# lixiny/ArtiBoost

Measured on AMD Instinct MI355X. Metric: synth samples/sec (render+fwd+bwd) 256x256 bs=64, higher is better.
Workload: dtype bf16x3; 1 GPU; train_artiboost HO3Dv2-clasbased (HybridBaseline/ResNet-34, 22x28x32x32 heat-map) + online CCV render 512->256, per-GPU batch 64, HO3D-like objects; global_batch=64, image=256, parallelism=dp1, graph=True, render_overlap=False

## Files before the change

artiboost_amd/csrc/conv_x3.hip:

```cpp
#include "conv_common.h"
#include "wgrad.h"

int conv3x3_x3_tiles(int N, int H, int W, int C, int Cn);
int conv3x3_x3_tiles_bnr(int N, int H, int W, int C, int Cn);
struct C3EvalBn { void* out_hi; void* out_lo; float* out_f32; const void* res_hi; const void* res_lo; int relu; };
int conv3x3_x3_run(const void* x_hi, const void* x_lo, const void* wt_hi, const void* wt_lo, float* out, int N, int H, int W,
                   int C, int Cn, int flip, const float* addend, float* stats, hipStream_t st, const float* bn_y = nullptr,
                   const void* bn_out_hi = nullptr, const float* bnp = nullptr, float* bn_part = nullptr, const C3EvalBn* ev = nullptr);
int conv_gemm2_x3_mtiles(int M, int Cn, int nsteps, int nclass);
int conv_gemm2_x3_run(ConvGemmArgs& g, hipStream_t st);
int conv_gemm2_x3_stem_mtiles(int M);
int conv_gemm2_x3_stem_run(ConvGemmArgs& g, hipStream_t st);
int stem_halo_x3_tiles(int N, int H, int W);
int stem_halo_x3_run(const void* xpad_hi, const void* xpad_lo, const void* w_hi, const void* w_lo, float* y, int N, int H, int W,
                     int Cout, float* stats, hipStream_t st);
int conv2x2_tfwd_rows(int N, int H, int W, int Cn, int K);
int conv2x2_tfwd_run(const void* x_hi, const void* x_lo, const void* wt_hi, const void* wt_lo, float* out, int N, int H, int W, int Cn, int K,
                     float* stats, hipStream_t st, const float* ep_scale = nullptr, const float* ep_shift = nullptr, int ep_relu = 0,
                     void* out_hi = nullptr, void* out_lo = nullptr);
int conv2x2_s2fwd_ok(int N, int H, int W, int C, int Cn);
int convp_s2fwd_rows(int N, int H, int W, int C, int Cn);
int convp_s2fwd_run(const void* x_hi, const void* x_lo, const void* w_hi, const void* w_lo, float* out, int N, int H, int W, int C, int Cn,
                    float* stats, hipStream_t st, const float* ep_scale = nullptr, const float* ep_shift = nullptr, int ep_relu = 0,
                    void* out_hi = nullptr, void* out_lo = nullptr);
// ... 316 lines not shown

extern "C" int ab_conv2d_wgrad_x3(const void* x_hi, const void* x_lo, const void* dy_hi, const void* dy_lo, float* dw, int N,
                                  int H, int W, int Cin, int Cout, int kh, int kw, int stride, int pad, void* workspace,
                                  int accumulate, void* stream) {
    if (!x_hi || !x_lo || !dy_hi || !dy_lo || !dw || !workspace) return AB_EINVAL;
    if (kh * kw > 16 || Cin % 64 || Cout % 64) return AB_ESHAPE;
    hipStream_t st = as_stream(stream);
    float* const slabs = (float*)workspace;
    const int jtot = kh * kw * Cin;
    if (x3_is_c3(kh, kw, stride, pad)) {
        if (int ns = wgrad3x3_x3_group_slices(1, N, H, W, Cin, Cout))
            return wgrad_then_reduce([&] { return wgrad3x3_x3_group_run(1, &x_hi, &x_lo, &dy_hi, &dy_lo, &slabs, N, H, W, Cin, Cout, st); },
                                     slabs, ns, Cout, jtot, jtot, dw, accumulate, 0, st);
    }
    {
        const long Ho = (H + 2 * pad - kh) / stride + 1, Wo = (W + 2 * pad - kw) / stride + 1;
        if ((long)N * Ho * Wo >= X3_WGRAD_MAX_M && N > 1) {
            const int n1 = N / 2;
            wgrad_reduce_now();
            const long xo = (long)n1 * H * W * Cin, yo = (long)n1 * Ho * Wo * Cout;
            int rc = ab_conv2d_wgrad_x3(x_hi, x_lo, dy_hi, dy_lo, dw, n1, H, W, Cin, Cout, kh, kw, stride, pad, workspace, accumulate, stream);
            if (rc) return rc;
            return ab_conv2d_wgrad_x3((const bf16_t*)x_hi + xo, (const bf16_t*)x_lo + xo, (const bf16_t*)dy_hi + yo, (const bf16_t*)dy_lo + yo,
                                      dw, N - n1, H, W, Cin, Cout, kh, kw, stride, pad, workspace, 1, stream);
        }
    }
    const int M = N * ((H + 2 * pad - kh) / stride + 1) * ((W + 2 * pad - kw) / stride + 1);
    int ns = wgrad_gemm2_x3_slices(M, Cout, Cin, kh * kw);
    if (ns <= 0) return AB_ESHAPE;
    return wgrad_then_reduce([&] { return wgrad_gemm2_x3_run(x_hi, x_lo, dy_hi, dy_lo, slabs, N, H, W, Cin, Cout, kh, kw, stride, pad, st); },
                             slabs, ns, Cout, jtot, jtot, dw, accumulate, 0, st);
}

extern "C" int ab_conv2d_stem_x3_stat_rows(int N, int H, int W) {
    if (int t = stem_halo_x3_tiles(N, H, W)) return t;
    return conv_gemm2_x3_stem_mtiles(N * (H / 2) * (W / 2));
}

extern "C" int ab_conv2d_stem_fwd_x3(const void* xpad_hi, const void* xpad_lo, const void* w_hi, const void* w_lo, float* y, int N,
                                     int H, int W, int Cout, float* stats, void* stream) {
    if (!xpad_hi || !w_hi || !w_lo || !y) return AB_EINVAL;
    if ((H & 1) || (W & 1) || Cout != 64) return AB_ESHAPE;
    if (stem_halo_x3_tiles(N, H, W)) return stem_halo_x3_run(xpad_hi, xpad_lo, w_hi, w_lo, y, N, H, W, Cout, stats, as_stream(stream));
    if (!xpad_lo) return AB_ESHAPE;
    ConvGemmArgs g = {};
    g.A = xpad_hi; g.A_lo = xpad_lo; g.Bw = w_hi; g.Bw_lo = w_lo; g.Out = y; g.stats = stats;
    g.N = N; g.Ha = H + 6; g.Wa = W + 8; g.Ca = 4;
    g.Ho = H / 2; g.Wo = W / 2; g.Cn = Cout; g.P = g.Ho; g.Q = g.Wo; g.out_sh = g.out_sw = 1; g.a_sh = g.a_sw = 2;
    g.ktot = 7 * 32; g.M = N * g.P * g.Q;
    return conv_gemm2_x3_stem_run(g, as_stream(stream));
}

static int stem_wgrad_x3_impl(const bf16_t* xpad_hi, const bf16_t* xpad_lo, const bf16_t* dy_hi, const bf16_t* dy_lo, float* dw, int N,
                              int H, int W, int Cout, void* workspace, int accumulate, hipStream_t st) {
    if ((long)N * (H / 2) * (W / 2) >= X3_WGRAD_MAX_M && N > 1) {
        const int n1 = N / 2;
        wgrad_reduce_now();
        const long xo = (long)n1 * (H + 6) * (W + 8) * 4, yo = (long)n1 * (H / 2) * (W / 2) * Cout;
        int rc = stem_wgrad_x3_impl(xpad_hi, xpad_lo, dy_hi, dy_lo, dw, n1, H, W, Cout, workspace, accumulate, st);
        if (rc) return rc;
        return stem_wgrad_x3_impl(xpad_hi + xo, xpad_lo ? xpad_lo + xo : nullptr, dy_hi + yo, dy_lo + yo, dw, N - n1, H, W, Cout, workspace, 1, st);
    }
    int ns = wgrad_gemm2_stem_slices(N, H, W, Cout);
    if (ns <= 0) return AB_ESHAPE;
    return wgrad_then_reduce([&] { return wgrad_gemm2_x3_stem_run(xpad_hi, xpad_lo, dy_hi, dy_lo, (float*)workspace, N, H, W, Cout, st); },
                             (float*)workspace, ns, Cout, 256, 7 * 32, dw, accumulate, 1, st);
// ... 10 lines not shown
```

artiboost_amd/csrc/torch_ops_gen.cpp:

```cpp
#include <ATen/ATen.h>
#include <c10/hip/HIPStream.h>
#include <torch/library.h>
#include "../../include/artiboost_hip.h"

static inline void* p(const c10::optional<at::Tensor>& t) { return (t.has_value() && t->defined()) ? t->data_ptr() : nullptr; }
static inline void* cur_stream() { return (void*)c10::hip::getCurrentHIPStream().stream(); }

#include <c10/hip/HIPFunctions.h>
typedef c10::optional<at::Tensor> OptT;
static inline bool has(const OptT& t) { return t.has_value() && t->defined(); }
static inline void ck_contig(const char* op, const char* a, const OptT& t) {
    if (has(t)) TORCH_CHECK(t->is_contiguous(), op, ": argument '", a, "' must be contiguous (the kernels take raw buffers)");
}
static inline void ck_dev(const char* op, const char* a, const OptT& t, int dt, bool contiguous) {
    if (!has(t)) return;
    TORCH_CHECK(t->is_cuda(), op, ": argument '", a, "' must be a HIP tensor, got a ", t->device().str(), " tensor");
    TORCH_CHECK(t->get_device() == c10::hip::current_device(), op, ": argument '", a, "' lives on device ", t->get_device(), ", the current device is ", (int)c10::hip::current_device());
    if (contiguous) TORCH_CHECK(t->is_contiguous(), op, ": argument '", a, "' must be contiguous (the kernel takes it as a raw buffer without a pitch)");
    if (dt >= 0) TORCH_CHECK((int)t->scalar_type() == dt, op, ": argument '", a, "' must be ", c10::toString((at::ScalarType)dt), ", got ", c10::toString(t->scalar_type()));
}
static inline void ck_host(const char* op, const char* a, const OptT& t) {
    if (!has(t)) return;
    TORCH_CHECK(t->is_cpu(), op, ": argument '", a, "' is a HOST structure / array of the C ABI and must be a CPU tensor, got a ", t->device().str(), " tensor");
    TORCH_CHECK(t->is_contiguous(), op, ": argument '", a, "' must be contiguous");
// ... 31 lines not shown
static void w_conv2d_stem_fwd(const c10::optional<at::Tensor>& xpad, const c10::optional<at::Tensor>& w, const c10::optional<at::Tensor>& y, int64_t dtype, int64_t N, int64_t H, int64_t W, int64_t Cout, const c10::optional<at::Tensor>& stats) { static const char* const OP = "artiboost_hip::conv2d_stem_fwd"; ck_dev(OP, "xpad", xpad, (int)-1, true); ck_dev(OP, "w", w, (int)-1, true); ck_dev(OP, "y", y, (int)-1, true); ck_dev(OP, "stats", stats, (int)at::kFloat, true); const long rc = (long)ab_conv2d_stem_fwd((const void*)p(xpad), (const void*)p(w), (void*)p(y), (int)dtype, (int)N, (int)H, (int)W, (int)Cout, (float*)p(stats), cur_stream()); TORCH_CHECK(rc == 0, "ab_conv2d_stem_fwd failed with code ", rc, rc > 0 ? " (hipError)" : " (argument error)"); }
static int64_t w_conv2d_dgrad_stat_rows(int64_t dtype, int64_t N, int64_t H, int64_t W, int64_t Cin, int64_t Cout, int64_t kh, int64_t kw, int64_t stride, int64_t pad) { return (int64_t)ab_conv2d_dgrad_stat_rows((int)dtype, (int)N, (int)H, (int)W, (int)Cin, (int)Cout, (int)kh, (int)kw, (int)stride, (int)pad); }
static void w_conv2d_dgrad(const c10::optional<at::Tensor>& dy, const c10::optional<at::Tensor>& wt, const c10::optional<at::Tensor>& dx, int64_t dtype, int64_t N, int64_t H, int64_t W, int64_t Cin, int64_t Cout, int64_t kh, int64_t kw, int64_t stride, int64_t pad, const c10::optional<at::Tensor>& addend, const c10::optional<at::Tensor>& stats) { static const char* const OP = "artiboost_hip::conv2d_dgrad"; ck_dev(OP, "dy", dy, (int)-1, true); ck_dev(OP, "wt", wt, (int)-1, true); ck_dev(OP, "dx", dx, (int)-1, true); ck_dev(OP, "addend", addend, (int)-1, true); ck_dev(OP, "stats", stats, (int)at::kFloat, true); ck_dtcode(OP, "dy", dy, dtype); ck_dtcode(OP, "wt", wt, dtype); ck_dtcode(OP, "dx", dx, dtype); ck_dtcode(OP, "addend", addend, dtype); ck_numel(OP, "dy", dy, (int64_t)(N*co(H,kh,stride,pad)*co(W,kw,stride,pad)*Cout)); ck_numel(OP, "wt", wt, (int64_t)(Cin*kh*kw*Cout)); ck_numel(OP, "dx", dx, (int64_t)(N*H*W*Cin)); ck_numel(OP, "addend", addend, (int64_t)(N*H*W*Cin)); const long rc = (long)ab_conv2d_dgrad((const void*)p(dy), (const void*)p(wt), (void*)p(dx), (int)dtype, (int)N, (int)H, (int)W, (int)Cin, (int)Cout, (int)kh, (int)kw, (int)stride, (int)pad, (const void*)p(addend), (float*)p(stats), cur_stream()); TORCH_CHECK(rc == 0, "ab_conv2d_dgrad failed with code ", rc, rc > 0 ? " (hipError)" : " (argument error)"); }
static int64_t w_conv2d_wgrad_workspace(int64_t M, int64_t Cout, int64_t jtot) { return (int64_t)ab_conv2d_wgrad_workspace((int)M, (int)Cout, (int)jtot); }
static void w_conv2d_wgrad(const c10::optional<at::Tensor>& x, const c10::optional<at::Tensor>& dy, const c10::optional<at::Tensor>& dw, int64_t dtype, int64_t N, int64_t H, int64_t W, int64_t Cin, int64_t Cout, int64_t kh, int64_t kw, int64_t stride, int64_t pad, const c10::optional<at::Tensor>& workspace, int64_t accumulate) { static const char* const OP = "artiboost_hip::conv2d_wgrad"; ck_dev(OP, "x", x, (int)-1, true); ck_dev(OP, "dy", dy, (int)-1, true); ck_dev(OP, "dw", dw, (int)at::kFloat, true); ck_dev(OP, "workspace", workspace, (int)-1, true); const long rc = (long)ab_conv2d_wgrad((const void*)p(x), (const void*)p(dy), (float*)p(dw), (int)dtype, (int)N, (int)H, (int)W, (int)Cin, (int)Cout, (int)kh, (int)kw, (int)stride, (int)pad, (void*)p(workspace), (int)accumulate, cur_stream()); TORCH_CHECK(rc == 0, "ab_conv2d_wgrad failed with code ", rc, rc > 0 ? " (hipError)" : " (argument error)"); }
static void w_conv2d_wgrad_deferred(const c10::optional<at::Tensor>& x, const c10::optional<at::Tensor>& dy, const c10::optional<at::Tensor>& dw, int64_t dtype, int64_t N, int64_t H, int64_t W, int64_t Cin, int64_t Cout, int64_t kh, int64_t kw, int64_t stride, int64_t pad, const c10::optional<at::Tensor>& workspace, int64_t accumulate, const c10::optional<at::Tensor>& pending) { static const char* const OP = "artiboost_hip::conv2d_wgrad_deferred"; ck_dev(OP, "x", x, (int)-1, true); ck_dev(OP, "dy", dy, (int)-1, true); ck_dev(OP, "dw", dw, (int)at::kFloat, true); ck_dev(OP, "workspace", workspace, (int)-1, true); ck_contig(OP, "pending", pending); const long rc = (long)ab_conv2d_wgrad_deferred((const void*)p(x), (const void*)p(dy), (float*)p(dw), (int)dtype, (int)N, (int)H, (int)W, (int)Cin, (int)Cout, (int)kh, (int)kw, (int)stride, (int)pad, (void*)p(workspace), (int)accumulate, (ab_wgrad_reduce_desc*)p(pending), cur_stream()); TORCH_CHECK(rc == 0, "ab_conv2d_wgrad_deferred failed with code ", rc, rc > 0 ? " (hipError)" : " (argument error)"); }
static void w_conv2d_stem_wgrad_deferred(const c10::optional<at::Tensor>& xpad, const c10::optional<at::Tensor>& dy, const c10::optional<at::Tensor>& dw, int64_t dtype, int64_t N, int64_t H, int64_t W, int64_t Cout, const c10::optional<at::Tensor>& workspace, const c10::optional<at::Tensor>& pending) { static const char* const OP = "artiboost_hip::conv2d_stem_wgrad_deferred"; ck_dev(OP, "xpad", xpad, (int)-1, true); ck_dev(OP, "dy", dy, (int)-1, true); ck_dev(OP, "dw", dw, (int)at::kFloat, true); ck_dev(OP, "workspace", workspace, (int)-1, true); ck_contig(OP, "pending", pending); const long rc = (long)ab_conv2d_stem_wgrad_deferred((const void*)p(xpad), (const void*)p(dy), (float*)p(dw), (int)dtype, (int)N, (int)H, (int)W, (int)Cout, (void*)p(workspace), (ab_wgrad_reduce_desc*)p(pending), cur_stream()); TORCH_CHECK(rc == 0, "ab_conv2d_stem_wgrad_deferred failed with code ", rc, rc > 0 ? " (hipError)" : " (argument error)"); }
static void w_conv2d_wgrad_x3_deferred(const c10::optional<at::Tensor>& x_hi, const c10::optional<at::Tensor>& x_lo, const c10::optional<at::Tensor>& dy_hi, const c10::optional<at::Tensor>& dy_lo, const c10::optional<at::Tensor>& dw, int64_t N, int64_t H, int64_t W, int64_t Cin, int64_t Cout, int64_t kh, int64_t kw, int64_t stride, int64_t pad, const c10::optional<at::Tensor>& workspace, int64_t accumulate, const c10::optional<at::Tensor>& pending) { static const char* const OP = "artiboost_hip::conv2d_wgrad_x3_deferred"; ck_dev(OP, "x_hi", x_hi, (int)-1, true); ck_dev(OP, "x_lo", x_lo, (int)-1, true); ck_dev(OP, "dy_hi", dy_hi, (int)-1, true); ck_dev(OP, "dy_lo", dy_lo, (int)-1, true); ck_dev(OP, "dw", dw, (int)at::kFloat, true); ck_dev(OP, "workspace", workspace, (int)-1, true); ck_contig(OP, "pending", pending); const long rc = (long)ab_conv2d_wgrad_x3_deferred((const void*)p(x_hi), (const void*)p(x_lo), (const void*)p(dy_hi), (const void*)p(dy_lo), (float*)p(dw), (int)N, (int)H, (int)W, (int)Cin, (int)Cout, (int)kh, (int)kw, (int)stride, (int)pad, (void*)p(workspace), (int)accumulate, (ab_wgrad_reduce_desc*)p(pending), cur_stream()); TORCH_CHECK(rc == 0, "ab_conv2d_wgrad_x3_deferred failed with code ", rc, rc > 0 ? " (hipError)" : " (argument error)"); }
static void w_conv2d_stem_wgrad_x3_deferred(const c10::optional<at::Tensor>& xpad_hi, const c10::optional<at::Tensor>& xpad_lo, const c10::optional<at::Tensor>& dy_hi, const c10::optional<at::Tensor>& dy_lo, const c10::optional<at::Tensor>& dw, int64_t N, int64_t H, int64_t W, int64_t Cout, const c10::optional<at::Tensor>& workspace, const c10::optional<at::Tensor>& pending) { static const char* const OP = "artiboost_hip::conv2d_stem_wgrad_x3_deferred"; ck_dev(OP, "xpad_hi", xpad_hi, (int)-1, true); ck_dev(OP, "xpad_lo", xpad_lo, (int)-1, true); ck_dev(OP, "dy_hi", dy_hi, (int)-1, true); ck_dev(OP, "dy_lo", dy_lo, (int)-1, true); ck_dev(OP, "dw", dw, (int)at::kFloat, true); ck_dev(OP, "workspace", workspace, (int)-1, true); ck_contig(OP, "pending", pending); const long rc = (long)ab_conv2d_stem_wgrad_x3_deferred((const void*)p(xpad_hi), (const void*)p(xpad_lo), (const void*)p(dy_hi), (const void*)p(dy_lo), (float*)p(dw), (int)N, (int)H, (int)W, (int)Cout, (void*)p(workspace), (ab_wgrad_reduce_desc*)p(pending), cur_stream()); TORCH_CHECK(rc == 0, "ab_conv2d_stem_wgrad_x3_deferred failed with code ", rc, rc > 0 ? " (hipError)" : " (argument error)"); }
static void w_wgrad_reduce_batch(const c10::optional<at::Tensor>& desc, int64_t n) { static const char* const OP = "artiboost_hip::wgrad_reduce_batch"; ck_contig(OP, "desc", desc); const long rc = (long)ab_wgrad_reduce_batch((const ab_wgrad_reduce_desc*)p(desc), (int)n, cur_stream()); TORCH_CHECK(rc == 0, "ab_wgrad_reduce_batch failed with code ", rc, rc > 0 ? " (hipError)" : " (argument error)"); }
static int64_t w_conv2d_wgrad_x3_group_workspace(int64_t G, int64_t N, int64_t H, int64_t W, int64_t Cin, int64_t Cout) { return (int64_t)ab_conv2d_wgrad_x3_group_workspace((int)G, (int)N, (int)H, (int)W, (int)Cin, (int)Cout); }
static void w_conv2d_wgrad_x3_group(const c10::optional<at::Tensor>& items_host, int64_t G, int64_t N, int64_t H, int64_t W, int64_t Cin, int64_t Cout, const c10::optional<at::Tensor>& workspace, int64_t accumulate) { static const char* const OP = "artiboost_hip::conv2d_wgrad_x3_group"; ck_host(OP, "items_host", items_host); ck_dev(OP, "workspace", workspace, (int)-1, true); ck_bytes(OP, "workspace", workspace, (int64_t)(ab_conv2d_wgrad_x3_group_workspace(G,N,H,W,Cin,Cout))); const long rc = (long)ab_conv2d_wgrad_x3_group((const ab_wgrad_group_item*)p(items_host), (int)G, (int)N, (int)H, (int)W, (int)Cin, (int)Cout, (void*)p(workspace), (int)accumulate, cur_stream()); TORCH_CHECK(rc == 0, "ab_conv2d_wgrad_x3_group failed with code ", rc, rc > 0 ? " (hipError)" : " (argument error)"); }
static int64_t w_conv2d_stem_wgrad_workspace(int64_t N, int64_t H, int64_t W, int64_t Cout) { return (int64_t)ab_conv2d_stem_wgrad_workspace((int)N, (int)H, (int)W, (int)Cout); }
static void w_conv2d_stem_wgrad(const c10::optional<at::Tensor>& xpad, const c10::optional<at::Tensor>& dy, const c10::optional<at::Tensor>& dw, int64_t dtype, int64_t N, int64_t H, int64_t W, int64_t Cout, const c10::optional<at::Tensor>& workspace) { static const char* const OP = "artiboost_hip::conv2d_stem_wgrad"; ck_dev(OP, "xpad", xpad, (int)-1, true); ck_dev(OP, "dy", dy, (int)-1, true); ck_dev(OP, "dw", dw, (int)at::kFloat, true); ck_dev(OP, "workspace", workspace, (int)-1, true); const long rc = (long)ab_conv2d_stem_wgrad((const void*)p(xpad), (const void*)p(dy), (float*)p(dw), (int)dtype, (int)N, (int)H, (int)W, (int)Cout, (void*)p(workspace), cur_stream()); TORCH_CHECK(rc == 0, "ab_conv2d_stem_wgrad failed with code ", rc, rc > 0 ? " (hipError)" : " (argument error)"); }
static void w_split_f32(const c10::optional<at::Tensor>& src, int64_t n, const c10::optional<at::Tensor>& hi, const c10::optional<at::Tensor>& lo) { static const char* const OP = "artiboost_hip::split_f32"; ck_dev(OP, "src", src, (int)at::kFloat, true); ck_dev(OP, "hi", hi, (int)-1, true); ck_dev(OP, "lo", lo, (int)-1, true); ck_dtype(OP, "hi", hi, at::kBFloat16); ck_dtype(OP, "lo", lo, at::kBFloat16); ck_numel(OP, "src", src, (int64_t)(n)); ck_numel(OP, "hi", hi, (int64_t)(n)); ck_numel(OP, "lo", lo, (int64_t)(n)); const long rc = (long)ab_split_f32((const float*)p(src), (long)n, (void*)p(hi), (void*)p(lo), cur_stream()); TORCH_CHECK(rc == 0, "ab_split_f32 failed with code ", rc, rc > 0 ? " (hipError)" : " (argument error)"); }
static int64_t w_conv2d_x3_stat_rows(int64_t N, int64_t H, int64_t W, int64_t Cin, int64_t Cout, int64_t kh, int64_t kw, int64_t stride, int64_t pad) { return (int64_t)ab_conv2d_x3_stat_rows((int)N, (int)H, (int)W, (int)Cin, (int)Cout, (int)kh, (int)kw, (int)stride, (int)pad); }
static void w_conv2d_fwd_x3(const c10::optional<at::Tensor>& x_hi, const c10::optional<at::Tensor>& x_lo, const c10::optional<at::Tensor>& w_hi, const c10::optional<at::Tensor>& w_lo, const c10::optional<at::Tensor>& y, int64_t N, int64_t H, int64_t W, int64_t Cin, int64_t Cout, int64_t kh, int64_t kw, int64_t stride, int64_t pad, const c10::optional<at::Tensor>& bias, const c10::optional<at::Tensor>& stats, int64_t relu) { static const char* const OP = "artiboost_hip::conv2d_fwd_x3"; ck_dev(OP, "x_hi", x_hi, (int)-1, true); ck_dev(OP, "x_lo", x_lo, (int)-1, true); ck_dev(OP, "w_hi", w_hi, (int)-1, true); ck_dev(OP, "w_lo", w_lo, (int)-1, true); ck_dev(OP, "y", y, (int)at::kFloat, true); ck_dev(OP, "bias", bias, (int)at::kFloat, true); ck_dev(OP, "stats", stats, (int)at::kFloat, true); ck_dtype(OP, "x_hi", x_hi, at::kBFloat16); ck_dtype(OP, "x_lo", x_lo, at::kBFloat16); ck_dtype(OP, "w_hi", w_hi, at::kBFloat16); ck_dtype(OP, "w_lo", w_lo, at::kBFloat16); ck_numel(OP, "x_hi", x_hi, (int64_t)(N*H*W*Cin)); ck_numel(OP, "x_lo", x_lo, (int64_t)(N*H*W*Cin)); ck_numel(OP, "w_hi", w_hi, (int64_t)(Cout*kh*kw*Cin)); ck_numel(OP, "w_lo", w_lo, (int64_t)(Cout*kh*kw*Cin)); ck_numel(OP, "y", y, (int64_t)(N*co(H,kh,stride,pad)*co(W,kw,stride,pad)*Cout)); ck_numel(OP, "bias", bias, (int64_t)(Cout)); ck_numel(OP, "stats", stats, (int64_t)(ab_conv2d_x3_stat_rows(N,H,W,Cin,Cout,kh,kw,stride,pad)*Cout*2)); const long rc = (long)ab_conv2d_fwd_x3((const void*)p(x_hi), (const void*)p(x_lo), (const void*)p(w_hi), (const void*)p(w_lo), (float*)p(y), (int)N, (int)H, (int)W, (int)Cin, (int)Cout, (int)kh, (int)kw, (int)stride, (int)pad, (const float*)p(bias), (float*)p(stats), (int)relu, cur_stream()); TORCH_CHECK(rc == 0, "ab_conv2d_fwd_x3 failed with code ", rc, rc > 0 ? " (hipError)" : " (argument error)"); }
static int64_t w_conv1x1_sam_fwd_x3_ok(int64_t B, int64_t H, int64_t W, int64_t Cin, int64_t C, int64_t D) { return (int64_t)ab_conv1x1_sam_fwd_x3_ok((int)B, (int)H, (int)W, (int)Cin, (int)C, (int)D); }
static void w_conv1x1_sam_fwd_x3(const c10::optional<at::Tensor>& x_hi, const c10::optional<at::Tensor>& x_lo, const c10::optional<at::Tensor>& w_hi, const c10::optional<at::Tensor>& w_lo, const c10::optional<at::Tensor>& bias, const c10::optional<at::Tensor>& logits, int64_t B, int64_t H, int64_t W, int64_t Cin, int64_t C, int64_t D, const c10::optional<at::Tensor>& part) { static const char* const OP = "artiboost_hip::conv1x1_sam_fwd_x3"; ck_dev(OP, "x_hi", x_hi, (int)-1, true); ck_dev(OP, "x_lo", x_lo, (int)-1, true); ck_dev(OP, "w_hi", w_hi, (int)-1, true); ck_dev(OP, "w_lo", w_lo, (int)-1, true); ck_dev(OP, "bias", bias, (int)at::kFloat, true); ck_dev(OP, "logits", logits, (int)at::kFloat, true); ck_dev(OP, "part", part, (int)at::kFloat, true); ck_dtype(OP, "x_hi", x_hi, at::kBFloat16); ck_dtype(OP, "x_lo", x_lo, at::kBFloat16); ck_dtype(OP, "w_hi", w_hi, at::kBFloat16); ck_dtype(OP, "w_lo", w_lo, at::kBFloat16); ck_numel(OP, "x_hi", x_hi, (int64_t)(B*H*W*Cin)); ck_numel(OP, "x_lo", x_lo, (int64_t)(B*H*W*Cin)); ck_numel(OP, "w_hi", w_hi, (int64_t)(C*32*Cin)); ck_numel(OP, "w_lo", w_lo, (int64_t)(C*32*Cin)); ck_numel(OP, "bias", bias, (int64_t)(C*32)); ck_numel(OP, "logits", logits, (int64_t)(B*H*W*C*32)); ck_numel(OP, "part", part, (int64_t)(B*(H*W/64)*C*8)); const long rc = (long)ab_conv1x1_sam_fwd_x3((const void*)p(x_hi), (const void*)p(x_lo), (const void*)p(w_hi), (const void*)p(w_lo), (const float*)p(bias), (float*)p(logits), (int)B, (int)H, (int)W, (int)Cin, (int)C, (int)D, (float*)p(part), cur_stream()); TORCH_CHECK(rc == 0, "ab_conv1x1_sam_fwd_x3 failed with code ", rc, rc > 0 ? " (hipError)" : " (argument error)"); }
static void w_softargmax3d_stage2(const c10::optional<at::Tensor>& part, int64_t B, int64_t C, int64_t ntile, const c10::optional<at::Tensor>& uvd, const c10::optional<at::Tensor>& conf, const c10::optional<at::Tensor>& stat) { static const char* const OP = "artiboost_hip::softargmax3d_stage2"; ck_dev(OP, "part", part, (int)at::kFloat, true); ck_dev(OP, "uvd", uvd, (int)at::kFloat, true); ck_dev(OP, "conf", conf, (int)at::kFloat, true); ck_dev(OP, "stat", stat, (int)at::kFloat, true); ck_numel(OP, "part", part, (int64_t)(B*ntile*C*8)); ck_numel(OP, "uvd", uvd, (int64_t)(B*C*3)); ck_numel(OP, "conf", conf, (int64_t)(B*C)); ck_numel(OP, "stat", stat, (int64_t)(B*C*2)); const long rc = (long)ab_softargmax3d_stage2((const float*)p(part), (int)B, (int)C, (int)ntile, (float*)p(uvd), (float*)p(conf), (float*)p(stat), cur_stream()); TORCH_CHECK(rc == 0, "ab_softargmax3d_stage2 failed with code ", rc, rc > 0 ? " (hipError)" : " (argument error)"); }
static int64_t w_conv2d_fwd_x3_evalbn_ok(int64_t N, int64_t H, int64_t W, int64_t Cin, int64_t Cout) { return (int64_t)ab_conv2d_fwd_x3_evalbn_ok((int)N, (int)H, (int)W, (int)Cin, (int)Cout); }
static void w_conv2d_fwd_x3_evalbn(const c10::optional<at::Tensor>& x_hi, const c10::optional<at::Tensor>& x_lo, const c10::optional<at::Tensor>& w_hi, const c10::optional<at::Tensor>& w_lo, int64_t N, int64_t H, int64_t W, int64_t Cin, int64_t Cout, const c10::optional<at::Tensor>& bnp, const c10::optional<at::Tensor>& res_hi, const c10::optional<at::Tensor>& res_lo, const c10::optional<at::Tensor>& res_f32, int64_t relu, const c10::optional<at::Tensor>& out_hi, const c10::optional<at::Tensor>& out_lo, const c10::optional<at::Tensor>& out_f32) { static const char* const OP = "artiboost_hip::conv2d_fwd_x3_evalbn"; ck_dev(OP, "x_hi", x_hi, (int)-1, true); ck_dev(OP, "x_lo", x_lo, (int)-1, true); ck_dev(OP, "w_hi", w_hi, (int)-1, true); ck_dev(OP, "w_lo", w_lo, (int)-1, true); ck_dev(OP, "bnp", bnp, (int)at::kFloat, true); ck_dev(OP, "res_hi", res_hi, (int)-1, true); ck_dev(OP, "res_lo", res_lo, (int)-1, true); ck_dev(OP, "res_f32", res_f32, (int)at::kFloat, true); ck_dev(OP, "out_hi", out_hi, (int)-1, true); ck_dev(OP, "out_lo", out_lo, (int)-1, true); ck_dev(OP, "out_f32", out_f32, (int)at::kFloat, true); ck_dtype(OP, "x_hi", x_hi, at::kBFloat16); ck_dtype(OP, "x_lo", x_lo, at::kBFloat16); ck_dtype(OP, "w_hi", w_hi, at::kBFloat16); ck_dtype(OP, "w_lo", w_lo, at::kBFloat16); ck_dtype(OP, "res_hi", res_hi, at::kBFloat16); ck_dtype(OP, "res_lo", res_lo, at::kBFloat16); ck_dtype(OP, "out_hi", out_hi, at::kBFloat16); ck_dtype(OP, "out_lo", out_lo, at::kBFloat16); ck_numel(OP, "x_hi", x_hi, (int64_t)(N*H*W*Cin)); ck_numel(OP, "x_lo", x_lo, (int64_t)(N*H*W*Cin)); ck_numel(OP, "w_hi", w_hi, (int64_t)(Cout*9*Cin)); ck_numel(OP, "w_lo", w_lo, (int64_t)(Cout*9*Cin)); ck_numel(OP, "bnp", bnp, (int64_t)(2*Cout)); ck_numel(OP, "res_hi", res_hi, (int64_t)(N*H*W*Cout)); ck_numel(OP, "res_lo", res_lo, (int64_t)(N*H*W*Cout)); ck_numel(OP, "res_f32", res_f32, (int64_t)(N*H*W*Cout)); ck_numel(OP, "out_hi", out_hi, (int64_t)(N*H*W*Cout)); ck_numel(OP, "out_lo", out_lo, (int64_t)(N*H*W*Cout)); ck_numel(OP, "out_f32", out_f32, (int64_t)(N*H*W*Cout)); const long rc = (long)ab_conv2d_fwd_x3_evalbn((const void*)p(x_hi), (const void*)p(x_lo), (const void*)p(w_hi), (const void*)p(w_lo), (int)N, (int)H, (int)W, (int)Cin, (int)Cout, (const float*)p(bnp), (const void*)p(res_hi), (const void*)p(res_lo), (const float*)p(res_f32), (int)relu, (void*)p(out_hi), (void*)p(out_lo), (float*)p(out_f32), cur_stream()); TORCH_CHECK(rc == 0, "ab_conv2d_fwd_x3_evalbn failed with code ", rc, rc > 0 ? " (hipError)" : " (argument error)"); }
static void w_conv2d_fwd_x3_affine(const c10::optional<at::Tensor>& x_hi, const c10::optional<at::Tensor>& x_lo, const c10::optional<at::Tensor>& w_hi, const c10::optional<at::Tensor>& w_lo, int64_t N, int64_t H, int64_t W, int64_t Cin, int64_t Cout, int64_t kh, int64_t kw, int64_t stride, int64_t pad, const c10::optional<at::Tensor>& scale, const c10::optional<at::Tensor>& shift, int64_t relu, const c10::optional<at::Tensor>& out_f32, const c10::optional<at::Tensor>& out_hi, const c10::optional<at::Tensor>& out_lo) { static const char* const OP = "artiboost_hip::conv2d_fwd_x3_affine"; ck_dev(OP, "x_hi", x_hi, (int)-1, true); ck_dev(OP, "x_lo", x_lo, (int)-1, true); ck_dev(OP, "w_hi", w_hi, (int)-1, true); ck_dev(OP, "w_lo", w_lo, (int)-1, true); ck_dev(OP, "scale", scale, (int)at::kFloat, true); ck_dev(OP, "shift", shift, (int)at::kFloat, true); ck_dev(OP, "out_f32", out_f32, (int)at::kFloat, true); ck_dev(OP, "out_hi", out_hi, (int)-1, true); ck_dev(OP, "out_lo", out_lo, (int)-1, true); ck_dtype(OP, "x_hi", x_hi, at::kBFloat16); ck_dtype(OP, "x_lo", x_lo, at::kBFloat16); ck_dtype(OP, "w_hi", w_hi, at::kBFloat16); ck_dtype(OP, "w_lo", w_lo, at::kBFloat16); ck_dtype(OP, "out_hi", out_hi, at::kBFloat16); ck_dtype(OP, "out_lo", out_lo, at::kBFloat16); ck_numel(OP, "x_hi", x_hi, (int64_t)(N*H*W*Cin)); ck_numel(OP, "x_lo", x_lo, (int64_t)(N*H*W*Cin)); ck_numel(OP, "w_hi", w_hi, (int64_t)(Cout*kh*kw*Cin)); ck_numel(OP, "w_lo", w_lo, (int64_t)(Cout*kh*kw*Cin)); ck_numel(OP, "scale", scale, (int64_t)(Cout)); ck_numel(OP, "shift", shift, (int64_t)(Cout)); ck_numel(OP, "out_f32", out_f32, (int64_t)(N*co(H,kh,stride,pad)*co(W,kw,stride,pad)*Cout)); ck_numel(OP, "out_hi", out_hi, (int64_t)(N*co(H,kh,stride,pad)*co(W,kw,stride,pad)*Cout)); ck_numel(OP, "out_lo", out_lo, (int64_t)(N*co(H,kh,stride,pad)*co(W,kw,stride,pad)*Cout)); const long rc = (long)ab_conv2d_fwd_x3_affine((const void*)p(x_hi), (const void*)p(x_lo), (const void*)p(w_hi), (const void*)p(w_lo), (int)N, (int)H, (int)W, (int)Cin, (int)Cout, (int)kh, (int)kw, (int)stride, (int)pad, (const float*)p(scale), (const float*)p(shift), (int)relu, (float*)p(out_f32), (void*)p(out_hi), (void*)p(out_lo), cur_stream()); TORCH_CHECK(rc == 0, "ab_conv2d_fwd_x3_affine failed with code ", rc, rc > 0 ? " (hipError)" : " (argument error)"); }
static void w_conv2d_dgrad_x3_affine(const c10::optional<at::Tensor>& dy_hi, const c10::optional<at::Tensor>& dy_lo, const c10::optional<at::Tensor>& wt_hi, const c10::optional<at::Tensor>& wt_lo, int64_t N, int64_t H, int64_t W, int64_t Cin, int64_t Cout, int64_t kh, int64_t kw, int64_t stride, int64_t pad, const c10::optional<at::Tensor>& scale, const c10::optional<at::Tensor>& shift, int64_t relu, const c10::optional<at::Tensor>& out_f32, const c10::optional<at::Tensor>& out_hi, const c10::optional<at::Tensor>& out_lo) { static const char* const OP = "artiboost_hip::conv2d_dgrad_x3_affine"; ck_dev(OP, "dy_hi", dy_hi, (int)-1, true); ck_dev(OP, "dy_lo", dy_lo, (int)-1, true); ck_dev(OP, "wt_hi", wt_hi, (int)-1, true); ck_dev(OP, "wt_lo", wt_lo, (int)-1, true); ck_dev(OP, "scale", scale, (int)at::kFloat, true); ck_dev(OP, "shift", shift, (int)at::kFloat, true); ck_dev(OP, "out_f32", out_f32, (int)at::kFloat, true); ck_dev(OP, "out_hi", out_hi, (int)-1, true); ck_dev(OP, "out_lo", out_lo, (int)-1, true); const long rc = (long)ab_conv2d_dgrad_x3_affine((const void*)p(dy_hi), (const void*)p(dy_lo), (const void*)p(wt_hi), (const void*)p(wt_lo), (int)N, (int)H, (int)W, (int)Cin, (int)Cout, (int)kh, (int)kw, (int)stride, (int)pad, (const float*)p(scale), (const float*)p(shift), (int)relu, (float*)p(out_f32), (void*)p(out_hi), (void*)p(out_lo), cur_stream()); TORCH_CHECK(rc == 0, "ab_conv2d_dgrad_x3_affine failed with code ", rc, rc > 0 ? " (hipError)" : " (argument error)"); }
static int64_t w_conv2d_dgrad_x3_stat_rows(int64_t N, int64_t H, int64_t W, int64_t Cin, int64_t Cout, int64_t kh, int64_t kw, int64_t stride, int64_t pad) { return (int64_t)ab_conv2d_dgrad_x3_stat_rows((int)N, (int)H, (int)W, (int)Cin, (int)Cout, (int)kh, (int)kw, (int)stride, (int)pad); }
static void w_conv2d_dgrad_x3(const c10::optional<at::Tensor>& dy_hi, const c10::optional<at::Tensor>& dy_lo, const c10::optional<at::Tensor>& wt_hi, const c10::optional<at::Tensor>& wt_lo, const c10::optional<at::Tensor>& dx, int64_t N, int64_t H, int64_t W, int64_t Cin, int64_t Cout, int64_t kh, int64_t kw, int64_t stride, int64_t pad, const c10::optional<at::Tensor>& addend, const c10::optional<at::Tensor>& stats) { static const char* const OP = "artiboost_hip::conv2d_dgrad_x3"; ck_dev(OP, "dy_hi", dy_hi, (int)-1, true); ck_dev(OP, "dy_lo", dy_lo, (int)-1, true); ck_dev(OP, "wt_hi", wt_hi, (int)-1, true); ck_dev(OP, "wt_lo", wt_lo, (int)-1, true); ck_dev(OP, "dx", dx, (int)at::kFloat, true); ck_dev(OP, "addend", addend, (int)at::kFloat, true); ck_dev(OP, "stats", stats, (int)at::kFloat, true); ck_dtype(OP, "dy_hi", dy_hi, at::kBFloat16); ck_dtype(OP, "dy_lo", dy_lo, at::kBFloat16); ck_dtype(OP, "wt_hi", wt_hi, at::kBFloat16); ck_dtype(OP, "wt_lo", wt_lo, at::kBFloat16); ck_numel(OP, "dy_hi", dy_hi, (int64_t)(N*co(H,kh,stride,pad)*co(W,kw,stride,pad)*Cout)); ck_numel(OP, "dy_lo", dy_lo, (int64_t)(N*co(H,kh,stride,pad)*co(W,kw,stride,pad)*Cout)); ck_numel(OP, "wt_hi", wt_hi, (int64_t)(Cin*kh*kw*Cout)); ck_numel(OP, "wt_lo", wt_lo, (int64_t)(Cin*kh*kw*Cout)); ck_numel(OP, "dx", dx, (int64_t)(N*H*W*Cin)); ck_numel(OP, "addend", addend, (int64_t)(N*H*W*Cin)); const long rc = (long)ab_conv2d_dgrad_x3((const void*)p(dy_hi), (const void*)p(dy_lo), (const void*)p(wt_hi), (const void*)p(wt_lo), (float*)p(dx), (int)N, (int)H, (int)W, (int)Cin, (int)Cout, (int)kh, (int)kw, (int)stride, (int)pad, (const float*)p(addend), (float*)p(stats), cur_stream()); TORCH_CHECK(rc == 0, "ab_conv2d_dgrad_x3 failed with code ", rc, rc > 0 ? " (hipError)" : " (argument error)"); }
static void w_conv2d_dgrad_x3_pair(const c10::optional<at::Tensor>& dy_hi, const c10::optional<at::Tensor>& dy_lo, const c10::optional<at::Tensor>& wt_hi, const c10::optional<at::Tensor>& wt_lo, const c10::optional<at::Tensor>& dy2_hi, const c10::optional<at::Tensor>& dy2_lo, const c10::optional<at::Tensor>& wt2_hi, const c10::optional<at::Tensor>& wt2_lo, const c10::optional<at::Tensor>& dx, int64_t N, int64_t H, int64_t W, int64_t Cin, int64_t Cout, int64_t kh, int64_t kw, int64_t pad, const c10::optional<at::Tensor>& addend) { static const char* const OP = "artiboost_hip::conv2d_dgrad_x3_pair"; ck_dev(OP, "dy_hi", dy_hi, (int)-1, true); ck_dev(OP, "dy_lo", dy_lo, (int)-1, true); ck_dev(OP, "wt_hi", wt_hi, (int)-1, true); ck_dev(OP, "wt_lo", wt_lo, (int)-1, true); ck_dev(OP, "dy2_hi", dy2_hi, (int)-1, true); ck_dev(OP, "dy2_lo", dy2_lo, (int)-1, true); ck_dev(OP, "wt2_hi", wt2_hi, (int)-1, true); ck_dev(OP, "wt2_lo", wt2_lo, (int)-1, true); ck_dev(OP, "dx", dx, (int)at::kFloat, true); ck_dev(OP, "addend", addend, (int)at::kFloat, true); ck_dtype(OP, "dy_hi", dy_hi, at::kBFloat16); ck_dtype(OP, "dy_lo", dy_lo, at::kBFloat16); ck_dtype(OP, "wt_hi", wt_hi, at::kBFloat16); ck_dtype(OP, "wt_lo", wt_lo, at::kBFloat16); ck_dtype(OP, "dy2_hi", dy2_hi, at::kBFloat16); ck_dtype(OP, "dy2_lo", dy2_lo, at::kBFloat16); ck_dtype(OP, "wt2_hi", wt2_hi, at::kBFloat16); ck_dtype(OP, "wt2_lo", wt2_lo, at::kBFloat16); ck_numel(OP, "dy_hi", dy_hi, (int64_t)(N*(H/2)*(W/2)*Cout)); ck_numel(OP, "dy_lo", dy_lo, (int64_t)(N*(H/2)*(W/2)*Cout)); ck_numel(OP, "dy2_hi", dy2_hi, (int64_t)(N*(H/2)*(W/2)*Cout)); ck_numel(OP, "dy2_lo", dy2_lo, (int64_t)(N*(H/2)*(W/2)*Cout)); ck_numel(OP, "wt_hi", wt_hi, (int64_t)(Cin*kh*kw*Cout)); ck_numel(OP, "wt_lo", wt_lo, (int64_t)(Cin*kh*kw*Cout)); ck_numel(OP, "wt2_hi", wt2_hi, (int64_t)(Cin*Cout)); ck_numel(OP, "wt2_lo", wt2_lo, (int64_t)(Cin*Cout)); ck_numel(OP, "dx", dx, (int64_t)(N*H*W*Cin)); ck_numel(OP, "addend", addend, (int64_t)(N*H*W*Cin)); const long rc = (long)ab_conv2d_dgrad_x3_pair((const void*)p(dy_hi), (const void*)p(dy_lo), (const void*)p(wt_hi), (const void*)p(wt_lo), (const void*)p(dy2_hi), (const void*)p(dy2_lo), (const void*)p(wt2_hi), (const void*)p(wt2_lo), (float*)p(dx), (int)N, (int)H, (int)W, (int)Cin, (int)Cout, (int)kh, (int)kw, (int)pad, (const float*)p(addend), cur_stream()); TORCH_CHECK(rc == 0, "ab_conv2d_dgrad_x3_pair failed with code ", rc, rc > 0 ? " (hipError)" : " (argument error)"); }
static int64_t w_conv2d_dgrad_x3_pair_bn_rows(int64_t N, int64_t H, int64_t W, int64_t Cin, int64_t Cout, int64_t kh, int64_t kw, int64_t pad) { return (int64_t)ab_conv2d_dgrad_x3_pair_bn_rows((int)N, (int)H, (int)W, (int)Cin, (int)Cout, (int)kh, (int)kw, (int)pad); }
static void w_conv2d_dgrad_x3_pair_bn(const c10::optional<at::Tensor>& dy_hi, const c10::optional<at::Tensor>& dy_lo, const c10::optional<at::Tensor>& wt_hi, const c10::optional<at::Tensor>& wt_lo, const c10::optional<at::Tensor>& dy2_hi, const c10::optional<at::Tensor>& dy2_lo, const c10::optional<at::Tensor>& wt2_hi, const c10::optional<at::Tensor>& wt2_lo, const c10::optional<at::Tensor>& dz, int64_t N, int64_t H, int64_t W, int64_t Cin, int64_t Cout, int64_t kh, int64_t kw, int64_t pad, const c10::optional<at::Tensor>& bn_y, const c10::optional<at::Tensor>& bn_out_hi, const c10::optional<at::Tensor>& bnp, const c10::optional<at::Tensor>& bn_part) { static const char* const OP = "artiboost_hip::conv2d_dgrad_x3_pair_bn"; ck_dev(OP, "dy_hi", dy_hi, (int)-1, true); ck_dev(OP, "dy_lo", dy_lo, (int)-1, true); ck_dev(OP, "wt_hi", wt_hi, (int)-1, true); ck_dev(OP, "wt_lo", wt_lo, (int)-1, true); ck_dev(OP, "dy2_hi", dy2_hi, (int)-1, true); ck_dev(OP, "dy2_lo", dy2_lo, (int)-1, true); ck_dev(OP, "wt2_hi", wt2_hi, (int)-1, true); ck_dev(OP, "wt2_lo", wt2_lo, (int)-1, true); ck_dev(OP, "dz", dz, (int)at::kFloat, true); ck_dev(OP, "bn_y", bn_y, (int)at::kFloat, true); ck_dev(OP, "bn_out_hi", bn_out_hi, (int)-1, true); ck_dev(OP, "bnp", bnp, (int)at::kFloat, true); ck_dev(OP, "bn_part", bn_part, (int)at::kFloat, true); ck_dtype(OP, "dy_hi", dy_hi, at::kBFloat16); ck_dtype(OP, "dy_lo", dy_lo, at::kBFloat16); ck_dtype(OP, "wt_hi", wt_hi, at::kBFloat16); ck_dtype(OP, "wt_lo", wt_lo, at::kBFloat16); ck_dtype(OP, "dy2_hi", dy2_hi, at::kBFloat16); ck_dtype(OP, "dy2_lo", dy2_lo, at::kBFloat16); ck_dtype(OP, "wt2_hi", wt2_hi, at::kBFloat16); ck_dtype(OP, "wt2_lo", wt2_lo, at::kBFloat16); ck_dtype(OP, "bn_out_hi", bn_out_hi, at::kBFloat16); ck_numel(OP, "dy_hi", dy_hi, (int64_t)(N*(H/2)*(W/2)*Cout)); ck_numel(OP, "dy_lo", dy_lo, (int64_t)(N*(H/2)*(W/2)*Cout)); ck_numel(OP, "dy2_hi", dy2_hi, (int64_t)(N*(H/2)*(W/2)*Cout)); ck_numel(OP, "dy2_lo", dy2_lo, (int64_t)(N*(H/2)*(W/2)*Cout)); ck_numel(OP, "wt_hi", wt_hi, (int64_t)(Cin*kh*kw*Cout)); ck_numel(OP, "wt_lo", wt_lo, (int64_t)(Cin*kh*kw*Cout)); ck_numel(OP, "wt2_hi", wt2_hi, (int64_t)(Cin*Cout)); ck_numel(OP, "wt2_lo", wt2_lo, (int64_t)(Cin*Cout)); ck_numel(OP, "dz", dz, (int64_t)(N*H*W*Cin)); ck_numel(OP, "bn_y", bn_y, (int64_t)(N*H*W*Cin)); ck_numel(OP, "bn_out_hi", bn_out_hi, (int64_t)(N*H*W*Cin)); ck_numel(OP, "bnp", bnp, (int64_t)(4*Cin)); ck_numel(OP, "bn_part", bn_part, (int64_t)(ab_conv2d_dgrad_x3_pair_bn_rows(N,H,W,Cin,Cout,kh,kw,pad)*Cin*2)); const long rc = (long)ab_conv2d_dgrad_x3_pair_bn((const void*)p(dy_hi), (const void*)p(dy_lo), (const void*)p(wt_hi), (const void*)p(wt_lo), (const void*)p(dy2_hi), (const void*)p(dy2_lo), (const void*)p(wt2_hi), (const void*)p(wt2_lo), (float*)p(dz), (int)N, (int)H, (int)W, (int)Cin, (int)Cout, (int)kh, (int)kw, (int)pad, (const float*)p(bn_y), (const void*)p(bn_out_hi), (const float*)p(bnp), (float*)p(bn_part), cur_stream()); TORCH_CHECK(rc == 0, "ab_conv2d_dgrad_x3_pair_bn failed with code ", rc, rc > 0 ? " (hipError)" : " (argument error)"); }
static int64_t w_conv2d_dgrad_x3_bn_rows(int64_t N, int64_t H, int64_t W, int64_t Cin, int64_t Cout, int64_t kh, int64_t kw, int64_t stride, int64_t pad) { return (int64_t)ab_conv2d_dgrad_x3_bn_rows((int)N, (int)H, (int)W, (int)Cin, (int)Cout, (int)kh, (int)kw, (int)stride, (int)pad); }
static void w_conv2d_dgrad_x3_bn(const c10::optional<at::Tensor>& dy_hi, const c10::optional<at::Tensor>& dy_lo, const c10::optional<at::Tensor>& wt_hi, const c10::optional<at::Tensor>& wt_lo, const c10::optional<at::Tensor>& dz, int64_t N, int64_t H, int64_t W, int64_t Cin, int64_t Cout, int64_t kh, int64_t kw, int64_t stride, int64_t pad, const c10::optional<at::Tensor>& addend, const c10::optional<at::Tensor>& bn_y, const c10::optional<at::Tensor>& bn_out_hi, const c10::optional<at::Tensor>& bnp, const c10::optional<at::Tensor>& bn_part) { static const char* const OP = "artiboost_hip::conv2d_dgrad_x3_bn"; ck_dev(OP, "dy_hi", dy_hi, (int)-1, true); ck_dev(OP, "dy_lo", dy_lo, (int)-1, true); ck_dev(OP, "wt_hi", wt_hi, (int)-1, true); ck_dev(OP, "wt_lo", wt_lo, (int)-1, true); ck_dev(OP, "dz", dz, (int)at::kFloat, true); ck_dev(OP, "addend", addend, (int)at::kFloat, true); ck_dev(OP, "bn_y", bn_y, (int)at::kFloat, true); ck_dev(OP, "bn_out_hi", bn_out_hi, (int)-1, true); ck_dev(OP, "bnp", bnp, (int)at::kFloat, true); ck_dev(OP, "bn_part", bn_part, (int)at::kFloat, true); ck_dtype(OP, "dy_hi", dy_hi, at::kBFloat16); ck_dtype(OP, "dy_lo", dy_lo, at::kBFloat16); ck_dtype(OP, "wt_hi", wt_hi, at::kBFloat16); ck_dtype(OP, "wt_lo", wt_lo, at::kBFloat16); ck_dtype(OP, "bn_out_hi", bn_out_hi, at::kBFloat16); ck_numel(OP, "dy_hi", dy_hi, (int64_t)(N*co(H,kh,stride,pad)*co(W,kw,stride,pad)*Cout)); ck_numel(OP, "dy_lo", dy_lo, (int64_t)(N*co(H,kh,stride,pad)*co(W,kw,stride,pad)*Cout)); ck_numel(OP, "wt_hi", wt_hi, (int64_t)(Cin*kh*kw*Cout)); ck_numel(OP, "wt_lo", wt_lo, (int64_t)(Cin*kh*kw*Cout)); ck_numel(OP, "dz", dz, (int64_t)(N*H*W*Cin)); ck_numel(OP, "addend", addend, (int64_t)(N*H*W*Cin)); ck_numel(OP, "bn_y", bn_y, (int64_t)(N*H*W*Cin)); ck_numel(OP, "bn_out_hi", bn_out_hi, (int64_t)(N*H*W*Cin)); ck_numel(OP, "bnp", bnp, (int64_t)(4*Cin)); ck_numel(OP, "bn_part", bn_part, (int64_t)(ab_conv2d_dgrad_x3_bn_rows(N,H,W,Cin,Cout,kh,kw,stride,pad)*Cin*2)); const long rc = (long)ab_conv2d_dgrad_x3_bn((const void*)p(dy_hi), (const void*)p(dy_lo), (const void*)p(wt_hi), (const void*)p(wt_lo), (float*)p(dz), (int)N, (int)H, (int)W, (int)Cin, (int)Cout, (int)kh, (int)kw, (int)stride, (int)pad, (const float*)p(addend), (const float*)p(bn_y), (const void*)p(bn_out_hi), (const float*)p(bnp), (float*)p(bn_part), cur_stream()); TORCH_CHECK(rc == 0, "ab_conv2d_dgrad_x3_bn failed with code ", rc, rc > 0 ? " (hipError)" : " (argument error)"); }
static int64_t w_conv2d_wgrad_x3_workspace(int64_t N, int64_t H, int64_t W, int64_t Cin, int64_t Cout, int64_t kh, int64_t kw, int64_t stride, int64_t pad) { return (int64_t)ab_conv2d_wgrad_x3_workspace((int)N, (int)H, (int)W, (int)Cin, (int)Cout, (int)kh, (int)kw, (int)stride, (int)pad); }
static void w_conv2d_wgrad_x3(const c10::optional<at::Tensor>& x_hi, const c10::optional<at::Tensor>& x_lo, const c10::optional<at::Tensor>& dy_hi, const c10::optional<at::Tensor>& dy_lo, const c10::optional<at::Tensor>& dw, int64_t N, int64_t H, int64_t W, int64_t Cin, int64_t Cout, int64_t kh, int64_t kw, int64_t stride, int64_t pad, const c10::optional<at::Tensor>& workspace, int64_t accumulate) { static const char* const OP = "artiboost_hip::conv2d_wgrad_x3"; ck_dev(OP, "x_hi", x_hi, (int)-1, true); ck_dev(OP, "x_lo", x_lo, (int)-1, true); ck_dev(OP, "dy_hi", dy_hi, (int)-1, true); ck_dev(OP, "dy_lo", dy_lo, (int)-1, true); ck_dev(OP, "dw", dw, (int)at::kFloat, true); ck_dev(OP, "workspace", workspace, (int)-1, true); ck_dtype(OP, "x_hi", x_hi, at::kBFloat16); ck_dtype(OP, "x_lo", x_lo, at::kBFloat16); ck_dtype(OP, "dy_hi", dy_hi, at::kBFloat16); ck_dtype(OP, "dy_lo", dy_lo, at::kBFloat16); ck_numel(OP, "x_hi", x_hi, (int64_t)(N*H*W*Cin)); ck_numel(OP, "x_lo", x_lo, (int64_t)(N*H*W*Cin)); ck_numel(OP, "dy_hi", dy_hi, (int64_t)(N*co(H,kh,stride,pad)*co(W,kw,stride,pad)*Cout)); ck_numel(OP, "dy_lo", dy_lo, (int64_t)(N*co(H,kh,stride,pad)*co(W,kw,stride,pad)*Cout)); ck_numel(OP, "dw", dw, (int64_t)(Cout*kh*kw*Cin)); ck_bytes(OP, "workspace", workspace, (int64_t)(ab_conv2d_wgrad_x3_workspace(N,H,W,Cin,Cout,kh,kw,stride,pad))); const long rc = (long)ab_conv2d_wgrad_x3((const void*)p(x_hi), (const void*)p(x_lo), (const void*)p(dy_hi), (const void*)p(dy_lo), (float*)p(dw), (int)N, (int)H, (int)W, (int)Cin, (int)Cout, (int)kh, (int)kw, (int)stride, (int)pad, (void*)p(workspace), (int)accumulate, cur_stream()); TORCH_CHECK(rc == 0, "ab_conv2d_wgrad_x3 failed with code ", rc, rc > 0 ? " (hipError)" : " (argument error)"); }
static int64_t w_conv2d_stem_x3_stat_rows(int64_t N, int64_t H, int64_t W) { return (int64_t)ab_conv2d_stem_x3_stat_rows((int)N, (int)H, (int)W); }
static void w_conv2d_stem_fwd_x3(const c10::optional<at::Tensor>& xpad_hi, const c10::optional<at::Tensor>& xpad_lo, const c10::optional<at::Tensor>& w_hi, const c10::optional<at::Tensor>& w_lo, const c10::optional<at::Tensor>& y, int64_t N, int64_t H, int64_t W, int64_t Cout, const c10::optional<at::Tensor>& stats) { static const char* const OP = "artiboost_hip::conv2d_stem_fwd_x3"; ck_dev(OP, "xpad_hi", xpad_hi, (int)-1, true); ck_dev(OP, "xpad_lo", xpad_lo, (int)-1, true); ck_dev(OP, "w_hi", w_hi, (int)-1, true); ck_dev(OP, "w_lo", w_lo, (int)-1, true); ck_dev(OP, "y", y, (int)at::kFloat, true); ck_dev(OP, "stats", stats, (int)at::kFloat, true); ck_dtype(OP, "xpad_hi", xpad_hi, at::kBFloat16); ck_dtype(OP, "xpad_lo", xpad_lo, at::kBFloat16); ck_dtype(OP, "w_hi", w_hi, at::kBFloat16); ck_dtype(OP, "w_lo", w_lo, at::kBFloat16); ck_numel(OP, "xpad_hi", xpad_hi, (int64_t)(N*(H+6)*(W+8)*4)); ck_numel(OP, "xpad_lo", xpad_lo, (int64_t)(N*(H+6)*(W+8)*4)); ck_numel(OP, "w_hi", w_hi, (int64_t)(Cout*7*8*4)); ck_numel(OP, "w_lo", w_lo, (int64_t)(Cout*7*8*4)); ck_numel(OP, "y", y, (int64_t)(N*(H/2)*(W/2)*Cout)); ck_numel(OP, "stats", stats, (int64_t)(ab_conv2d_stem_x3_stat_rows(N,H,W)*Cout*2)); const long rc = (long)ab_conv2d_stem_fwd_x3((const void*)p(xpad_hi), (const void*)p(xpad_lo), (const void*)p(w_hi), (const void*)p(w_lo), (float*)p(y), (int)N, (int)H, (int)W, (int)Cout, (float*)p(stats), cur_stream()); TORCH_CHECK(rc == 0, "ab_conv2d_stem_fwd_x3 failed with code ", rc, rc > 0 ? " (hipError)" : " (argument error)"); }
static void w_conv2d_stem_wgrad_x3(const c10::optional<at::Tensor>& xpad_hi, const c10::optional<at::Tensor>& xpad_lo, const c10::optional<at::Tensor>& dy_hi, const c10::optional<at::Tensor>& dy_lo, const c10::optional<at::Tensor>& dw, int64_t N, int64_t H, int64_t W, int64_t Cout, const c10::optional<at::Tensor>& workspace) { static const char* const OP = "artiboost_hip::conv2d_stem_wgrad_x3"; ck_dev(OP, "xpad_hi", xpad_hi, (int)-1, true); ck_dev(OP, "xpad_lo", xpad_lo, (int)-1, true); ck_dev(OP, "dy_hi", dy_hi, (int)-1, true); ck_dev(OP, "dy_lo", dy_lo, (int)-1, true); ck_dev(OP, "dw", dw, (int)at::kFloat, true); ck_dev(OP, "workspace", workspace, (int)-1, true); ck_dtype(OP, "xpad_hi", xpad_hi, at::kBFloat16); ck_dtype(OP, "xpad_lo", xpad_lo, at::kBFloat16); ck_dtype(OP, "dy_hi", dy_hi, at::kBFloat16); ck_dtype(OP, "dy_lo", dy_lo, at::kBFloat16); ck_numel(OP, "xpad_hi", xpad_hi, (int64_t)(N*(H+6)*(W+8)*4)); ck_numel(OP, "xpad_lo", xpad_lo, (int64_t)(N*(H+6)*(W+8)*4)); ck_numel(OP, "dy_hi", dy_hi, (int64_t)(N*(H/2)*(W/2)*Cout)); ck_numel(OP, "dy_lo", dy_lo, (int64_t)(N*(H/2)*(W/2)*Cout)); ck_numel(OP, "dw", dw, (int64_t)(Cout*7*8*4)); const long rc = (long)ab_conv2d_stem_wgrad_x3((const void*)p(xpad_hi), (const void*)p(xpad_lo), (const void*)p(dy_hi), (const void*)p(dy_lo), (float*)p(dw), (int)N, (int)H, (int)W, (int)Cout, (void*)p(workspace), cur_stream()); TORCH_CHECK(rc == 0, "ab_conv2d_stem_wgrad_x3 failed with code ", rc, rc > 0 ? " (hipError)" : " (argument error)"); }
static void w_bn_apply_x3(const c10::optional<at::Tensor>& y, const c10::optional<at::Tensor>& res, const c10::optional<at::Tensor>& bnp, int64_t M, int64_t C, int64_t relu, const c10::optional<at::Tensor>& out, const c10::optional<at::Tensor>& out_hi, const c10::optional<at::Tensor>& out_lo) { static const char* const OP = "artiboost_hip::bn_apply_x3"; ck_dev(OP, "y", y, (int)at::kFloat, true); ck_dev(OP, "res", res, (int)at::kFloat, true); ck_dev(OP, "bnp", bnp, (int)at::kFloat, true); ck_dev(OP, "out", out, (int)at::kFloat, true); ck_dev(OP, "out_hi", out_hi, (int)-1, true); ck_dev(OP, "out_lo", out_lo, (int)-1, true); ck_dtype(OP, "out_hi", out_hi, at::kBFloat16); ck_dtype(OP, "out_lo", out_lo, at::kBFloat16); ck_numel(OP, "y", y, (int64_t)(M*C)); ck_numel(OP, "res", res, (int64_t)(M*C)); ck_numel(OP, "out", out, (int64_t)(M*C)); ck_numel(OP, "out_hi", out_hi, (int64_t)(M*C)); ck_numel(OP, "out_lo", out_lo, (int64_t)(M*C)); ck_numel(OP, "bnp", bnp, (int64_t)(2*C)); const long rc = (long)ab_bn_apply_x3((const float*)p(y), (const float*)p(res), (const float*)p(bnp), (long)M, (int)C, (int)relu, (float*)p(out), (void*)p(out_hi), (void*)p(out_lo), cur_stream()); TORCH_CHECK(rc == 0, "ab_bn_apply_x3 failed with code ", rc, rc > 0 ? " (hipError)" : " (argument error)"); }
static void w_bn_apply_x3_resbn(const c10::optional<at::Tensor>& y, const c10::optional<at::Tensor>& res_y, const c10::optional<at::Tensor>& bnp, const c10::optional<at::Tensor>& res_bnp, int64_t M, int64_t C, int64_t relu, const c10::optional<at::Tensor>& out, const c10::optional<at::Tensor>& out_hi, const c10::optional<at::Tensor>& out_lo) { static const char* const OP = "artiboost_hip::bn_apply_x3_resbn"; ck_dev(OP, "y", y, (int)at::kFloat, true); ck_dev(OP, "res_y", res_y, (int)at::kFloat, true); ck_dev(OP, "bnp", bnp, (int)at::kFloat, true); ck_dev(OP, "res_bnp", res_bnp, (int)at::kFloat, true); ck_dev(OP, "out", out, (int)at::kFloat, true); ck_dev(OP, "out_hi", out_hi, (int)-1, true); ck_dev(OP, "out_lo", out_lo, (int)-1, true); const long rc = (long)ab_bn_apply_x3_resbn((const float*)p(y), (const float*)p(res_y), (const float*)p(bnp), (const float*)p(res_bnp), (long)M, (int)C, (int)relu, (float*)p(out), (void*)p(out_hi), (void*)p(out_lo), cur_stream()); TORCH_CHECK(rc == 0, "ab_bn_apply_x3_resbn failed with code ", rc, rc > 0 ? " (hipError)" : " (argument error)"); }
static void w_bn_apply_x3_respl(const c10::optional<at::Tensor>& y, const c10::optional<at::Tensor>& res_hi, const c10::optional<at::Tensor>& res_lo, const c10::optional<at::Tensor>& bnp, int64_t M, int64_t C, int64_t relu, const c10::optional<at::Tensor>& out, const c10::optional<at::Tensor>& out_hi, const c10::optional<at::Tensor>& out_lo) { static const char* const OP = "artiboost_hip::bn_apply_x3_respl"; ck_dev(OP, "y", y, (int)at::kFloat, true); ck_dev(OP, "res_hi", res_hi, (int)-1, true); ck_dev(OP, "res_lo", res_lo, (int)-1, true); ck_dev(OP, "bnp", bnp, (int)at::kFloat, true); ck_dev(OP, "out", out, (int)at::kFloat, true); ck_dev(OP, "out_hi", out_hi, (int)-1, true); ck_dev(OP, "out_lo", out_lo, (int)-1, true); ck_dtype(OP, "res_hi", res_hi, at::kBFloat16); ck_dtype(OP, "res_lo", res_lo, at::kBFloat16); ck_dtype(OP, "out_hi", out_hi, at::kBFloat16); ck_dtype(OP, "out_lo", out_lo, at::kBFloat16); ck_numel(OP, "y", y, (int64_t)(M*C)); ck_numel(OP, "res_hi", res_hi, (int64_t)(M*C)); ck_numel(OP, "res_lo", res_lo, (int64_t)(M*C)); ck_numel(OP, "out", out, (int64_t)(M*C)); ck_numel(OP, "out_hi", out_hi, (int64_t)(M*C)); ck_numel(OP, "out_lo", out_lo, (int64_t)(M*C)); ck_numel(OP, "bnp", bnp, (int64_t)(2*C)); const long rc = (long)ab_bn_apply_x3_respl((const float*)p(y), (const void*)p(res_hi), (const void*)p(res_lo), (const float*)p(bnp), (long)M, (int)C, (int)relu, (float*)p(out), (void*)p(out_hi), (void*)p(out_lo), cur_stream()); TORCH_CHECK(rc == 0, "ab_bn_apply_x3_respl failed with code ", rc, rc > 0 ? " (hipError)" : " (argument error)"); }
static int64_t w_bn_fin_apply_x3_ok(int64_t nparts, int64_t C) { return (int64_t)ab_bn_fin_apply_x3_ok((int)nparts, (int)C); }
static void w_bn_fin_apply_x3(const c10::optional<at::Tensor>& part, int64_t nparts, int64_t count, const c10::optional<at::Tensor>& gamma, const c10::optional<at::Tensor>& beta, double eps, double momentum, const c10::optional<at::Tensor>& running_mean, const c10::optional<at::Tensor>& running_var, const c10::optional<at::Tensor>& bnp, const c10::optional<at::Tensor>& y, const c10::optional<at::Tensor>& res, const c10::optional<at::Tensor>& res_hi, const c10::optional<at::Tensor>& res_lo, const c10::optional<at::Tensor>& res_bnp, int64_t M, int64_t C, int64_t relu, const c10::optional<at::Tensor>& out, const c10::optional<at::Tensor>& out_hi, const c10::optional<at::Tensor>& out_lo) { static const char* const OP = "artiboost_hip::bn_fin_apply_x3"; ck_dev(OP, "part", part, (int)at::kFloat, true); ck_dev(OP, "gamma", gamma, (int)at::kFloat, true); ck_dev(OP, "beta", beta, (int)at::kFloat, true); ck_dev(OP, "running_mean", running_mean, (int)at::kFloat, true); ck_dev(OP, "running_var", running_var, (int)at::kFloat, true); ck_dev(OP, "bnp", bnp, (int)at::kFloat, true); ck_dev(OP, "y", y, (int)at::kFloat, true); ck_dev(OP, "res", res, (int)at::kFloat, true); ck_dev(OP, "res_hi", res_hi, (int)-1, true); ck_dev(OP, "res_lo", res_lo, (int)-1, true); ck_dev(OP, "res_bnp", res_bnp, (int)at::kFloat, true); ck_dev(OP, "out", out, (int)at::kFloat, true); ck_dev(OP, "out_hi", out_hi, (int)-1, true); ck_dev(OP, "out_lo", out_lo, (int)-1, true); ck_dtype(OP, "res_hi", res_hi, at::kBFloat16); ck_dtype(OP, "res_lo", res_lo, at::kBFloat16); ck_dtype(OP, "out_hi", out_hi, at::kBFloat16); ck_dtype(OP, "out_lo", out_lo, at::kBFloat16); ck_numel(OP, "part", part, (int64_t)(nparts*C*2)); ck_numel(OP, "gamma", gamma, (int64_t)(C)); ck_numel(OP, "beta", beta, (int64_t)(C)); ck_numel(OP, "running_mean", running_mean, (int64_t)(C)); ck_numel(OP, "running_var", running_var, (int64_t)(C)); ck_numel(OP, "bnp", bnp, (int64_t)(4*C)); ck_numel(OP, "res_bnp", res_bnp, (int64_t)(2*C)); ck_numel(OP, "y", y, (int64_t)(M*C)); ck_numel(OP, "res", res, (int64_t)(M*C)); ck_numel(OP, "res_hi", res_hi, (int64_t)(M*C)); ck_numel(OP, "res_lo", res_lo, (int64_t)(M*C)); ck_numel(OP, "out", out, (int64_t)(M*C)); ck_numel(OP, "out_hi", out_hi, (int64_t)(M*C)); ck_numel(OP, "out_lo", out_lo, (int64_t)(M*C)); const long rc = (long)ab_bn_fin_apply_x3((const float*)p(part), (int)nparts, (long)count, (const float*)p(gamma), (const float*)p(beta), (float)eps, (float)momentum, (float*)p(running_mean), (float*)p(running_var), (float*)p(bnp), (const float*)p(y), (const float*)p(res), (const void*)p(res_hi), (const void*)p(res_lo), (const float*)p(res_bnp), (long)M, (int)C, (int)relu, (float*)p(out), (void*)p(out_hi), (void*)p(out_lo), cur_stream()); TORCH_CHECK(rc == 0, "ab_bn_fin_apply_x3 failed with code ", rc, rc > 0 ? " (hipError)" : " (argument error)"); }
static void w_bn_bwd_x3(const c10::optional<at::Tensor>& dout, const c10::optional<at::Tensor>& out, int64_t out_is_hi_plane, const c10::optional<at::Tensor>& y, const c10::optional<at::Tensor>& bnp, int64_t M, int64_t C, int64_t relu, const c10::optional<at::Tensor>& part, int64_t nparts_given, const c10::optional<at::Tensor>& bwdp, const c10::optional<at::Tensor>& dgamma, const c10::optional<at::Tensor>& dbeta, const c10::optional<at::Tensor>& dy_hi, const c10::optional<at::Tensor>& dy_lo, const c10::optional<at::Tensor>& dz_out) { static const char* const OP = "artiboost_hip::bn_bwd_x3"; ck_dev(OP, "dout", dout, (int)at::kFloat, true); ck_dev(OP, "out", out, (int)-1, true); ck_dev(OP, "y", y, (int)at::kFloat, true); ck_dev(OP, "bnp", bnp, (int)at::kFloat, true); ck_dev(OP, "part", part, (int)at::kFloat, true); ck_dev(OP, "bwdp", bwdp, (int)at::kFloat, true); ck_dev(OP, "dgamma", dgamma, (int)at::kFloat, true); ck_dev(OP, "dbeta", dbeta, (int)at::kFloat, true); ck_dev(OP, "dy_hi", dy_hi, (int)-1, true); ck_dev(OP, "dy_lo", dy_lo, (int)-1, true); ck_dev(OP, "dz_out", dz_out, (int)at::kFloat, true); ck_dtype(OP, "dy_hi", dy_hi, at::kBFloat16); ck_dtype(OP, "dy_lo", dy_lo, at::kBFloat16); ck_numel(OP, "dout", dout, (int64_t)(M*C)); ck_numel(OP, "y", y, (int64_t)(M*C)); ck_numel(OP, "dy_hi", dy_hi, (int64_t)(M*C)); ck_numel(OP, "dy_lo", dy_lo, (int64_t)(M*C)); ck_numel(OP, "dz_out", dz_out, (int64_t)(M*C)); ck_numel(OP, "bnp", bnp, (int64_t)(4*C)); ck_numel(OP, "dgamma", dgamma, (int64_t)(C)); ck_numel(OP, "dbeta", dbeta, (int64_t)(C)); const long rc = (long)ab_bn_bwd_x3((const float*)p(dout), (const void*)p(out), (int)out_is_hi_plane, (const float*)p(y), (const float*)p(bnp), (long)M, (int)C, (int)relu, (float*)p(part), (int)nparts_given, (float*)p(bwdp), (float*)p(dgamma), (float*)p(dbeta), (void*)p(dy_hi), (void*)p(dy_lo), (float*)p(dz_out), cur_stream()); TORCH_CHECK(rc == 0, "ab_bn_bwd_x3 failed with code ", rc, rc > 0 ? " (hipError)" : " (argument error)"); }
static int64_t w_col_stats_nparts(int64_t M) { return (int64_t)ab_col_stats_nparts((long)M); }
static void w_col_stats(const c10::optional<at::Tensor>& x, int64_t dtype, int64_t M, int64_t C, const c10::optional<at::Tensor>& part) { static const char* const OP = "artiboost_hip::col_stats"; ck_dev(OP, "x", x, (int)-1, true); ck_dev(OP, "part", part, (int)at::kFloat, true); ck_dtcode(OP, "x", x, dtype); ck_numel(OP, "x", x, (int64_t)(M*C)); ck_numel(OP, "part", part, (int64_t)(ab_col_stats_nparts(M)*C*2)); const long rc = (long)ab_col_stats((const void*)p(x), (int)dtype, (long)M, (int)C, (float*)p(part), cur_stream()); TORCH_CHECK(rc == 0, "ab_col_stats failed with code ", rc, rc > 0 ? " (hipError)" : " (argument error)"); }
static void w_bn_finalize(const c10::optional<at::Tensor>& part, int64_t nparts, int64_t C, int64_t count, const c10::optional<at::Tensor>& gamma, const c10::optional<at::Tensor>& beta, double eps, double momentum, const c10::optional<at::Tensor>& running_mean, const c10::optional<at::Tensor>& running_var, const c10::optional<at::Tensor>& bnp) { static const char* const OP = "artiboost_hip::bn_finalize"; ck_dev(OP, "part", part, (int)at::kFloat, true); ck_dev(OP, "gamma", gamma, (int)at::kFloat, true); ck_dev(OP, "beta", beta, (int)at::kFloat, true); ck_dev(OP, "running_mean", running_mean, (int)at::kFloat, true); ck_dev(OP, "running_var", running_var, (int)at::kFloat, true); ck_dev(OP, "bnp", bnp, (int)at::kFloat, true); ck_numel(OP, "part", part, (int64_t)(nparts*C*2)); ck_numel(OP, "gamma", gamma, (int64_t)(C)); ck_numel(OP, "beta", beta, (int64_t)(C)); ck_numel(OP, "running_mean", running_mean, (int64_t)(C)); ck_numel(OP, "running_var", running_var, (int64_t)(C)); ck_numel(OP, "bnp", bnp, (int64_t)(4*C)); const long rc = (long)ab_bn_finalize((const float*)p(part), (int)nparts, (int)C, (long)count, (const float*)p(gamma), (const float*)p(beta), (float)eps, (float)momentum, (float*)p(running_mean), (float*)p(running_var), (float*)p(bnp), cur_stream()); TORCH_CHECK(rc == 0, "ab_bn_finalize failed with code ", rc, rc > 0 ? " (hipError)" : " (argument error)"); }
static void w_bn_eval_params(int64_t C, const c10::optional<at::Tensor>& gamma, const c10::optional<at::Tensor>& beta, const c10::optional<at::Tensor>& rm, const c10::optional<at::Tensor>& rv, double eps, const c10::optional<at::Tensor>& bnp) { static const char* const OP = "artiboost_hip::bn_eval_params"; ck_dev(OP, "gamma", gamma, (int)at::kFloat, true); ck_dev(OP, "beta", beta, (int)at::kFloat, true); ck_dev(OP, "rm", rm, (int)at::kFloat, true); ck_dev(OP, "rv", rv, (int)at::kFloat, true); ck_dev(OP, "bnp", bnp, (int)at::kFloat, true); ck_numel(OP, "gamma", gamma, (int64_t)(C)); ck_numel(OP, "beta", beta, (int64_t)(C)); ck_numel(OP, "rm", rm, (int64_t)(C)); ck_numel(OP, "rv", rv, (int64_t)(C)); ck_numel(OP, "bnp", bnp, (int64_t)(4*C)); const long rc = (long)ab_bn_eval_params((int)C, (const float*)p(gamma), (const float*)p(beta), (const float*)p(rm), (const float*)p(rv), (float)eps, (float*)p(bnp), cur_stream()); TORCH_CHECK(rc == 0, "ab_bn_eval_params failed with code ", rc, rc > 0 ? " (hipError)" : " (argument error)"); }
static void w_bn_eval_params_batch(const c10::optional<at::Tensor>& flat, const c10::optional<at::Tensor>& stats, const c10::optional<at::Tensor>& desc_dev, int64_t n, int64_t max_c, double eps, const c10::optional<at::Tensor>& out) { static const char* const OP = "artiboost_hip::bn_eval_params_batch"; ck_dev(OP, "flat", flat, (int)at::kFloat, true); ck_dev(OP, "stats", stats, (int)at::kFloat, true); ck_dev(OP, "desc_dev", desc_dev, (int)at::kInt, true); ck_dev(OP, "out", out, (int)at::kFloat, true); const long rc = (long)ab_bn_eval_params_batch((const float*)p(flat), (const float*)p(stats), (const int32_t*)p(desc_dev), (int)n, (int)max_c, (float)eps, (float*)p(out), cur_stream()); TORCH_CHECK(rc == 0, "ab_bn_eval_params_batch failed with code ", rc, rc > 0 ? " (hipError)" : " (argument error)"); }
static void w_bn_apply(const c10::optional<at::Tensor>& y, const c10::optional<at::Tensor>& res, const c10::optional<at::Tensor>& bnp, int64_t dtype, int64_t M, int64_t C, int64_t relu, const c10::optional<at::Tensor>& out) { static const char* const OP = "artiboost_hip::bn_apply"; ck_dev(OP, "y", y, (int)-1, true); ck_dev(OP, "res", res, (int)-1, true); ck_dev(OP, "bnp", bnp, (int)at::kFloat, true); ck_dev(OP, "out", out, (int)-1, true); const long rc = (long)ab_bn_apply((const void*)p(y), (const void*)p(res), (const float*)p(bnp), (int)dtype, (long)M, (int)C, (int)relu, (void*)p(out), cur_stream()); TORCH_CHECK(rc == 0, "ab_bn_apply failed with code ", rc, rc > 0 ? " (hipError)" : " (argument error)"); }
static void w_bn_bwd(const c10::optional<at::Tensor>& dout, const c10::optional<at::Tensor>& out, const c10::optional<at::Tensor>& y, const c10::optional<at::Tensor>& bnp, int64_t dtype, int64_t M, int64_t C, int64_t relu, const c10::optional<at::Tensor>& part, const c10::optional<at::Tensor>& bwdp, const c10::optional<at::Tensor>& dgamma, const c10::optional<at::Tensor>& dbeta, const c10::optional<at::Tensor>& dy, const c10::optional<at::Tensor>& dz_out) { static const char* const OP = "artiboost_hip::bn_bwd"; ck_dev(OP, "dout", dout, (int)-1, true); ck_dev(OP, "out", out, (int)-1, true); ck_dev(OP, "y", y, (int)-1, true); ck_dev(OP, "bnp", bnp, (int)at::kFloat, true); ck_dev(OP, "part", part, (int)at::kFloat, true); ck_dev(OP, "bwdp", bwdp, (int)at::kFloat, true); ck_dev(OP, "dgamma", dgamma, (int)at::kFloat, true); ck_dev(OP, "dbeta", dbeta, (int)at::kFloat, true); ck_dev(OP, "dy", dy, (int)-1, true); ck_dev(OP, "dz_out", dz_out, (int)-1, true); const long rc = (long)ab_bn_bwd((const void*)p(dout), (const void*)p(out), (const void*)p(y), (const float*)p(bnp), (int)dtype, (long)M, (int)C, (int)relu, (float*)p(part), (float*)p(bwdp), (float*)p(dgamma), (float*)p(dbeta), (void*)p(dy), (void*)p(dz_out), cur_stream()); TORCH_CHECK(rc == 0, "ab_bn_bwd failed with code ", rc, rc > 0 ? " (hipError)" : " (argument error)"); }
static void w_relu_bwd(const c10::optional<at::Tensor>& dout, const c10::optional<at::Tensor>& out, int64_t dtype, int64_t n, const c10::optional<at::Tensor>& dz) { static const char* const OP = "artiboost_hip::relu_bwd"; ck_dev(OP, "dout", dout, (int)-1, true); ck_dev(OP, "out", out, (int)-1, true); ck_dev(OP, "dz", dz, (int)-1, true); const long rc = (long)ab_relu_bwd((const void*)p(dout), (const void*)p(out), (int)dtype, (long)n, (void*)p(dz), cur_stream()); TORCH_CHECK(rc == 0, "ab_relu_bwd failed with code ", rc, rc > 0 ? " (hipError)" : " (argument error)"); }
static void w_col_sum(const c10::optional<at::Tensor>& x, int64_t dtype, int64_t M, int64_t C, const c10::optional<at::Tensor>& part, const c10::optional<at::Tensor>& out) { static const char* const OP = "artiboost_hip::col_sum"; ck_dev(OP, "x", x, (int)-1, true); ck_dev(OP, "part", part, (int)at::kFloat, true); ck_dev(OP, "out", out, (int)at::kFloat, true); const long rc = (long)ab_col_sum((const void*)p(x), (int)dtype, (long)M, (int)C, (float*)p(part), (float*)p(out), cur_stream()); TORCH_CHECK(rc == 0, "ab_col_sum failed with code ", rc, rc > 0 ? " (hipError)" : " (argument error)"); }
static void w_col_sum_x3(const c10::optional<at::Tensor>& hi, const c10::optional<at::Tensor>& lo, int64_t M, int64_t C, const c10::optional<at::Tensor>& part, const c10::optional<at::Tensor>& out) { static const char* const OP = "artiboost_hip::col_sum_x3"; ck_dev(OP, "hi", hi, (int)-1, true); ck_dev(OP, "lo", lo, (int)-1, true); ck_dev(OP, "part", part, (int)at::kFloat, true); ck_dev(OP, "out", out, (int)at::kFloat, true); const long rc = (long)ab_col_sum_x3((const void*)p(hi), (const void*)p(lo), (long)M, (int)C, (float*)p(part), (float*)p(out), cur_stream()); TORCH_CHECK(rc == 0, "ab_col_sum_x3 failed with code ", rc, rc > 0 ? " (hipError)" : " (argument error)"); }
static void w_add(const c10::optional<at::Tensor>& a, const c10::optional<at::Tensor>& b, int64_t dtype, int64_t n, const c10::optional<at::Tensor>& out) { static const char* const OP = "artiboost_hip::add"; ck_dev(OP, "a", a, (int)-1, true); ck_dev(OP, "b", b, (int)-1, true); ck_dev(OP, "out", out, (int)-1, true); const long rc = (long)ab_add((const void*)p(a), (const void*)p(b), (int)dtype, (long)n, (void*)p(out), cur_stream()); TORCH_CHECK(rc == 0, "ab_add failed with code ", rc, rc > 0 ? " (hipError)" : " (argument error)"); }
static void w_maxpool3x3s2_fwd(const c10::optional<at::Tensor>& x, int64_t dtype, int64_t N, int64_t H, int64_t W, int64_t C, const c10::optional<at::Tensor>& out, const c10::optional<at::Tensor>& idx) { static const char* const OP = "artiboost_hip::maxpool3x3s2_fwd"; ck_dev(OP, "x", x, (int)-1, true); ck_dev(OP, "out", out, (int)-1, true); ck_dev(OP, "idx", idx, (int)-1, true); const long rc = (long)ab_maxpool3x3s2_fwd((const void*)p(x), (int)dtype, (int)N, (int)H, (int)W, (int)C, (void*)p(out), (void*)p(idx), cur_stream()); TORCH_CHECK(rc == 0, "ab_maxpool3x3s2_fwd failed with code ", rc, rc > 0 ? " (hipError)" : " (argument error)"); }
static int64_t w_conv2d_dgrad_bnstats_rows(int64_t dtype, int64_t N, int64_t H, int64_t W, int64_t Cin, int64_t Cout, int64_t kh, int64_t kw, int64_t stride, int64_t pad) { return (int64_t)ab_conv2d_dgrad_bnstats_rows((int)dtype, (int)N, (int)H, (int)W, (int)Cin, (int)Cout, (int)kh, (int)kw, (int)stride, (int)pad); }
static void w_conv2d_dgrad_bnstats(const c10::optional<at::Tensor>& dy, const c10::optional<at::Tensor>& wt, const c10::optional<at::Tensor>& dx, int64_t dtype, int64_t N, int64_t H, int64_t W, int64_t Cin, int64_t Cout, int64_t kh, int64_t kw, int64_t stride, int64_t pad, const c10::optional<at::Tensor>& addend, const c10::optional<at::Tensor>& bn_y, const c10::optional<at::Tensor>& bn_out, const c10::optional<at::Tensor>& bnp, const c10::optional<at::Tensor>& bn_part) { static const char* const OP = "artiboost_hip::conv2d_dgrad_bnstats"; ck_dev(OP, "dy", dy, (int)-1, true); ck_dev(OP, "wt", wt, (int)-1, true); ck_dev(OP, "dx", dx, (int)-1, true); ck_dev(OP, "addend", addend, (int)-1, true); ck_dev(OP, "bn_y", bn_y, (int)-1, true); ck_dev(OP, "bn_out", bn_out, (int)-1, true); ck_dev(OP, "bnp", bnp, (int)at::kFloat, true); ck_dev(OP, "bn_part", bn_part, (int)at::kFloat, true); const long rc = (long)ab_conv2d_dgrad_bnstats((const void*)p(dy), (const void*)p(wt), (void*)p(dx), (int)dtype, (int)N, (int)H, (int)W, (int)Cin, (int)Cout, (int)kh, (int)kw, (int)stride, (int)pad, (const void*)p(addend), (const void*)p(bn_y), (const void*)p(bn_out), (const float*)p(bnp), (float*)p(bn_part), cur_stream()); TORCH_CHECK(rc == 0, "ab_conv2d_dgrad_bnstats failed with code ", rc, rc > 0 ? " (hipError)" : " (argument error)"); }
static void w_bn_bwd_apply(const c10::optional<at::Tensor>& dout, const c10::optional<at::Tensor>& out, const c10::optional<at::Tensor>& y, const c10::optional<at::Tensor>& bnp, int64_t dtype, int64_t M, int64_t C, int64_t relu, const c10::optional<at::Tensor>& part, int64_t nparts, const c10::optional<at::Tensor>& bwdp, const c10::optional<at::Tensor>& dgamma, const c10::optional<at::Tensor>& dbeta, const c10::optional<at::Tensor>& dy, const c10::optional<at::Tensor>& dz_out) { static const char* const OP = "artiboost_hip::bn_bwd_apply"; ck_dev(OP, "dout", dout, (int)-1, true); ck_dev(OP, "out", out, (int)-1, true); ck_dev(OP, "y", y, (int)-1, true); ck_dev(OP, "bnp", bnp, (int)at::kFloat, true); ck_dev(OP, "part", part, (int)at::kFloat, true); ck_dev(OP, "bwdp", bwdp, (int)at::kFloat, true); ck_dev(OP, "dgamma", dgamma, (int)at::kFloat, true); ck_dev(OP, "dbeta", dbeta, (int)at::kFloat, true); ck_dev(OP, "dy", dy, (int)-1, true); ck_dev(OP, "dz_out", dz_out, (int)-1, true); const long rc = (long)ab_bn_bwd_apply((const void*)p(dout), (const void*)p(out), (const void*)p(y), (const float*)p(bnp), (int)dtype, (long)M, (int)C, (int)relu, (const float*)p(part), (int)nparts, (float*)p(bwdp), (float*)p(dgamma), (float*)p(dbeta), (void*)p(dy), (void*)p(dz_out), cur_stream()); TORCH_CHECK(rc == 0, "ab_bn_bwd_apply failed with code ", rc, rc > 0 ? " (hipError)" : " (argument error)"); }
static void w_bn_relu_maxpool3x3s2_fwd(const c10::optional<at::Tensor>& y, const c10::optional<at::Tensor>& bnp, int64_t dtype, int64_t N, int64_t H, int64_t W, int64_t C, const c10::optional<at::Tensor>& out, const c10::optional<at::Tensor>& idx) { static const char* const OP = "artiboost_hip::bn_relu_maxpool3x3s2_fwd"; ck_dev(OP, "y", y, (int)-1, true); ck_dev(OP, "bnp", bnp, (int)at::kFloat, true); ck_dev(OP, "out", out, (int)-1, true); ck_dev(OP, "idx", idx, (int)-1, true); const long rc = (long)ab_bn_relu_maxpool3x3s2_fwd((const void*)p(y), (const float*)p(bnp), (int)dtype, (int)N, (int)H, (int)W, (int)C, (void*)p(out), (void*)p(idx), cur_stream()); TORCH_CHECK(rc == 0, "ab_bn_relu_maxpool3x3s2_fwd failed with code ", rc, rc > 0 ? " (hipError)" : " (argument error)"); }
static void w_bn_relu_maxpool3x3s2_fwd_x3(const c10::optional<at::Tensor>& y, const c10::optional<at::Tensor>& bnp, int64_t N, int64_t H, int64_t W, int64_t C, const c10::optional<at::Tensor>& out, const c10::optional<at::Tensor>& out_hi, const c10::optional<at::Tensor>& out_lo, const c10::optional<at::Tensor>& idx) { static const char* const OP = "artiboost_hip::bn_relu_maxpool3x3s2_fwd_x3"; ck_dev(OP, "y", y, (int)at::kFloat, true); ck_dev(OP, "bnp", bnp, (int)at::kFloat, true); ck_dev(OP, "out", out, (int)at::kFloat, true); ck_dev(OP, "out_hi", out_hi, (int)-1, true); ck_dev(OP, "out_lo", out_lo, (int)-1, true); ck_dev(OP, "idx", idx, (int)-1, true); const long rc = (long)ab_bn_relu_maxpool3x3s2_fwd_x3((const float*)p(y), (const float*)p(bnp), (int)N, (int)H, (int)W, (int)C, (float*)p(out), (void*)p(out_hi), (void*)p(out_lo), (void*)p(idx), cur_stream()); TORCH_CHECK(rc == 0, "ab_bn_relu_maxpool3x3s2_fwd_x3 failed with code ", rc, rc > 0 ? " (hipError)" : " (argument error)"); }
static void w_bn_relu_maxpool_bwd(const c10::optional<at::Tensor>& dpool, const c10::optional<at::Tensor>& idx, const c10::optional<at::Tensor>& y, const c10::optional<at::Tensor>& bnp, int64_t dtype, int64_t N, int64_t H, int64_t W, int64_t C, const c10::optional<at::Tensor>& part, const c10::optional<at::Tensor>& bwdp, const c10::optional<at::Tensor>& dgamma, const c10::optional<at::Tensor>& dbeta, const c10::optional<at::Tensor>& dy) { static const char* const OP = "artiboost_hip::bn_relu_maxpool_bwd"; ck_dev(OP, "dpool", dpool, (int)-1, true); ck_dev(OP, "idx", idx, (int)-1, true); ck_dev(OP, "y", y, (int)-1, true); ck_dev(OP, "bnp", bnp, (int)at::kFloat, true); ck_dev(OP, "part", part, (int)at::kFloat, true); ck_dev(OP, "bwdp", bwdp, (int)at::kFloat, true); ck_dev(OP, "dgamma", dgamma, (int)at::kFloat, true); ck_dev(OP, "dbeta", dbeta, (int)at::kFloat, true); ck_dev(OP, "dy", dy, (int)-1, true); const long rc = (long)ab_bn_relu_maxpool_bwd((const void*)p(dpool), (const void*)p(idx), (const void*)p(y), (const float*)p(bnp), (int)dtype, (int)N, (int)H, (int)W, (int)C, (float*)p(part), (float*)p(bwdp), (float*)p(dgamma), (float*)p(dbeta), (void*)p(dy), cur_stream()); TORCH_CHECK(rc == 0, "ab_bn_relu_maxpool_bwd failed with code ", rc, rc > 0 ? " (hipError)" : " (argument error)"); }
static int64_t w_bn_relu_maxpool_bwd_x3_nparts(int64_t N, int64_t H, int64_t W, int64_t C) { return (int64_t)ab_bn_relu_maxpool_bwd_x3_nparts((int)N, (int)H, (int)W, (int)C); }
static void w_bn_relu_maxpool_bwd_x3(const c10::optional<at::Tensor>& dpool, const c10::optional<at::Tensor>& idx, const c10::optional<at::Tensor>& y, const c10::optional<at::Tensor>& bnp, int64_t N, int64_t H, int64_t W, int64_t C, const c10::optional<at::Tensor>& part, const c10::optional<at::Tensor>& bwdp, const c10::optional<at::Tensor>& dgamma, const c10::optional<at::Tensor>& dbeta, const c10::optional<at::Tensor>& dz, const c10::optional<at::Tensor>& dy_hi, const c10::optional<at::Tensor>& dy_lo) { static const char* const OP = "artiboost_hip::bn_relu_maxpool_bwd_x3"; ck_dev(OP, "dpool", dpool, (int)at::kFloat, true); ck_dev(OP, "idx", idx, (int)-1, true); ck_dev(OP, "y", y, (int)at::kFloat, true); ck_dev(OP, "bnp", bnp, (int)at::kFloat, true); ck_dev(OP, "part", part, (int)at::kFloat, true); ck_dev(OP, "bwdp", bwdp, (int)at::kFloat, true); ck_dev(OP, "dgamma", dgamma, (int)at::kFloat, true); ck_dev(OP, "dbeta", dbeta, (int)at::kFloat, true); ck_dev(OP, "dz", dz, (int)at::kFloat, true); ck_dev(OP, "dy_hi", dy_hi, (int)-1, true); ck_dev(OP, "dy_lo", dy_lo, (int)-1, true); const long rc = (long)ab_bn_relu_maxpool_bwd_x3((const float*)p(dpool), (const void*)p(idx), (const float*)p(y), (const float*)p(bnp), (int)N, (int)H, (int)W, (int)C, (float*)p(part), (float*)p(bwdp), (float*)p(dgamma), (float*)p(dbeta), (float*)p(dz), (void*)p(dy_hi), (void*)p(dy_lo), cur_stream()); TORCH_CHECK(rc == 0, "ab_bn_relu_maxpool_bwd_x3 failed with code ", rc, rc > 0 ? " (hipError)" : " (argument error)"); }
static void w_bn_relu_maxpool3x3s2_fwd_x3w(const c10::optional<at::Tensor>& y, const c10::optional<at::Tensor>& bnp, int64_t N, int64_t H, int64_t W, int64_t C, const c10::optional<at::Tensor>& out, const c10::optional<at::Tensor>& out_hi, const c10::optional<at::Tensor>& out_lo, const c10::optional<at::Tensor>& idx, const c10::optional<at::Tensor>& ywin) { static const char* const OP = "artiboost_hip::bn_relu_maxpool3x3s2_fwd_x3w"; ck_dev(OP, "y", y, (int)at::kFloat, true); ck_dev(OP, "bnp", bnp, (int)at::kFloat, true); ck_dev(OP, "out", out, (int)at::kFloat, true); ck_dev(OP, "out_hi", out_hi, (int)-1, true); ck_dev(OP, "out_lo", out_lo, (int)-1, true); ck_dev(OP, "idx", idx, (int)-1, true); ck_dev(OP, "ywin", ywin, (int)at::kFloat, true); ck_dtype(OP, "out_hi", out_hi, at::kBFloat16); ck_dtype(OP, "out_lo", out_lo, at::kBFloat16); ck_numel(OP, "y", y, (int64_t)(N*H*W*C)); ck_numel(OP, "bnp", bnp, (int64_t)(2*C)); ck_numel(OP, "out", out, (int64_t)(N*(H/2)*(W/2)*C)); ck_numel(OP, "out_hi", out_hi, (int64_t)(N*(H/2)*(W/2)*C)); ck_numel(OP, "out_lo", out_lo, (int64_t)(N*(H/2)*(W/2)*C)); ck_numel(OP, "ywin", ywin, (int64_t)(N*(H/2)*(W/2)*C)); ck_bytes(OP, "idx", idx, (int64_t)(N*(H/2)*(W/2)*C)); const long rc = (long)ab_bn_relu_maxpool3x3s2_fwd_x3w((const float*)p(y), (const float*)p(bnp), (int)N, (int)H, (int)W, (int)C, (float*)p(out), (void*)p(out_hi), (void*)p(out_lo), (void*)p(idx), (float*)p(ywin), cur_stream()); TORCH_CHECK(rc == 0, "ab_bn_relu_maxpool3x3s2_fwd_x3w failed with code ", rc, rc > 0 ? " (hipError)" : " (argument error)"); }
static void w_bn_relu_maxpool_bwd_x3w(const c10::optional<at::Tensor>& dpool, const c10::optional<at::Tensor>& idx, const c10::optional<at::Tensor>& ywin, const c10::optional<at::Tensor>& y, const c10::optional<at::Tensor>& bnp, int64_t N, int64_t H, int64_t W, int64_t C, const c10::optional<at::Tensor>& part, const c10::optional<at::Tensor>& bwdp, const c10::optional<at::Tensor>& dgamma, const c10::optional<at::Tensor>& dbeta, const c10::optional<at::Tensor>& dy_hi, const c10::optional<at::Tensor>& dy_lo) { static const char* const OP = "artiboost_hip::bn_relu_maxpool_bwd_x3w"; ck_dev(OP, "dpool", dpool, (int)at::kFloat, true); ck_dev(OP, "idx", idx, (int)-1, true); ck_dev(OP, "ywin", ywin, (int)at::kFloat, true); ck_dev(OP, "y", y, (int)at::kFloat, true); ck_dev(OP, "bnp", bnp, (int)at::kFloat, true); ck_dev(OP, "part", part, (int)at::kFloat, true); ck_dev(OP, "bwdp", bwdp, (int)at::kFloat, true); ck_dev(OP, "dgamma", dgamma, (int)at::kFloat, true); ck_dev(OP, "dbeta", dbeta, (int)at::kFloat, true); ck_dev(OP, "dy_hi", dy_hi, (int)-1, true); ck_dev(OP, "dy_lo", dy_lo, (int)-1, true); const long rc = (long)ab_bn_relu_maxpool_bwd_x3w((const float*)p(dpool), (const void*)p(idx), (const float*)p(ywin), (const float*)p(y), (const float*)p(bnp), (int)N, (int)H, (int)W, (int)C, (float*)p(part), (float*)p(bwdp), (float*)p(dgamma), (float*)p(dbeta), (void*)p(dy_hi), (void*)p(dy_lo), cur_stream()); TORCH_CHECK(rc == 0, "ab_bn_relu_maxpool_bwd_x3w failed with code ", rc, rc > 0 ? " (hipError)" : " (argument error)"); }
static void w_maxpool3x3s2_bwd(const c10::optional<at::Tensor>& idx, const c10::optional<at::Tensor>& dout, int64_t dtype, int64_t N, int64_t H, int64_t W, int64_t C, const c10::optional<at::Tensor>& dx) { static const char* const OP = "artiboost_hip::maxpool3x3s2_bwd"; ck_dev(OP, "idx", idx, (int)-1, true); ck_dev(OP, "dout", dout, (int)-1, true); ck_dev(OP, "dx", dx, (int)-1, true); const long rc = (long)ab_maxpool3x3s2_bwd((const void*)p(idx), (const void*)p(dout), (int)dtype, (int)N, (int)H, (int)W, (int)C, (void*)p(dx), cur_stream()); TORCH_CHECK(rc == 0, "ab_maxpool3x3s2_bwd failed with code ", rc, rc > 0 ? " (hipError)" : " (argument error)"); }
static void w_avgpool_fwd(const c10::optional<at::Tensor>& x, int64_t dtype, int64_t N, int64_t HW, int64_t C, const c10::optional<at::Tensor>& out) { static const char* const OP = "artiboost_hip::avgpool_fwd"; ck_dev(OP, "x", x, (int)-1, true); ck_dev(OP, "out", out, (int)at::kFloat, true); ck_dtcode(OP, "x", x, dtype); ck_numel(OP, "x", x, (int64_t)(N*HW*C)); ck_numel(OP, "out", out, (int64_t)(N*C)); const long rc = (long)ab_avgpool_fwd((const void*)p(x), (int)dtype, (int)N, (int)HW, (int)C, (float*)p(out), cur_stream()); TORCH_CHECK(rc == 0, "ab_avgpool_fwd failed with code ", rc, rc > 0 ? " (hipError)" : " (argument error)"); }
// ... 122 lines not shown
    m.def("conv2d_stem_fwd(Tensor? xpad, Tensor? w, Tensor(a!)? y, int dtype, int N, int H, int W, int Cout, Tensor(b!)? stats) -> ()");
    m.def("conv2d_dgrad_stat_rows(int dtype, int N, int H, int W, int Cin, int Cout, int kh, int kw, int stride, int pad) -> int");
    m.def("conv2d_dgrad(Tensor? dy, Tensor? wt, Tensor(a!)? dx, int dtype, int N, int H, int W, int Cin, int Cout, int kh, int kw, int stride, int pad, Tensor? addend, Tensor(b!)? stats) -> ()");
    m.def("conv2d_wgrad_workspace(int M, int Cout, int jtot) -> int");
    m.def("conv2d_wgrad(Tensor? x, Tensor? dy, Tensor(a!)? dw, int dtype, int N, int H, int W, int Cin, int Cout, int kh, int kw, int stride, int pad, Tensor(b!)? workspace, int accumulate) -> ()");
    m.def("conv2d_wgrad_deferred(Tensor? x, Tensor? dy, Tensor(a!)? dw, int dtype, int N, int H, int W, int Cin, int Cout, int kh, int kw, int stride, int pad, Tensor(b!)? workspace, int accumulate, Tensor(c!)? pending) -> ()");
    m.def("conv2d_stem_wgrad_deferred(Tensor? xpad, Tensor? dy, Tensor(a!)? dw, int dtype, int N, int H, int W, int Cout, Tensor(b!)? workspace, Tensor(c!)? pending) -> ()");
    m.def("conv2d_wgrad_x3_deferred(Tensor? x_hi, Tensor? x_lo, Tensor? dy_hi, Tensor? dy_lo, Tensor(a!)? dw, int N, int H, int W, int Cin, int Cout, int kh, int kw, int stride, int pad, Tensor(b!)? workspace, int accumulate, Tensor(c!)? pending) -> ()");
    m.def("conv2d_stem_wgrad_x3_deferred(Tensor? xpad_hi, Tensor? xpad_lo, Tensor? dy_hi, Tensor? dy_lo, Tensor(a!)? dw, int N, int H, int W, int Cout, Tensor(b!)? workspace, Tensor(c!)? pending) -> ()");
    m.def("wgrad_reduce_batch(Tensor? desc, int n) -> ()");
    m.def("conv2d_wgrad_x3_group_workspace(int G, int N, int H, int W, int Cin, int Cout) -> int");
    m.def("conv2d_wgrad_x3_group(Tensor? items_host, int G, int N, int H, int W, int Cin, int Cout, Tensor(a!)? workspace, int accumulate) -> ()");
    m.def("conv2d_stem_wgrad_workspace(int N, int H, int W, int Cout) -> int");
    m.def("conv2d_stem_wgrad(Tensor? xpad, Tensor? dy, Tensor(a!)? dw, int dtype, int N, int H, int W, int Cout, Tensor(b!)? workspace) -> ()");
    m.def("split_f32(Tensor? src, int n, Tensor(a!)? hi, Tensor(b!)? lo) -> ()");
    m.def("conv2d_x3_stat_rows(int N, int H, int W, int Cin, int Cout, int kh, int kw, int stride, int pad) -> int");
    m.def("conv2d_fwd_x3(Tensor? x_hi, Tensor? x_lo, Tensor? w_hi, Tensor? w_lo, Tensor(a!)? y, int N, int H, int W, int Cin, int Cout, int kh, int kw, int stride, int pad, Tensor? bias, Tensor(b!)? stats, int relu) -> ()");
    m.def("conv1x1_sam_fwd_x3_ok(int B, int H, int W, int Cin, int C, int D) -> int");
    m.def("conv1x1_sam_fwd_x3(Tensor? x_hi, Tensor? x_lo, Tensor? w_hi, Tensor? w_lo, Tensor? bias, Tensor(a!)? logits, int B, int H, int W, int Cin, int C, int D, Tensor(b!)? part) -> ()");
    m.def("softargmax3d_stage2(Tensor? part, int B, int C, int ntile, Tensor(a!)? uvd, Tensor(b!)? conf, Tensor(c!)? stat) -> ()");
    m.def("conv2d_fwd_x3_evalbn_ok(int N, int H, int W, int Cin, int Cout) -> int");
    m.def("conv2d_fwd_x3_evalbn(Tensor? x_hi, Tensor? x_lo, Tensor? w_hi, Tensor? w_lo, int N, int H, int W, int Cin, int Cout, Tensor? bnp, Tensor? res_hi, Tensor? res_lo, Tensor? res_f32, int relu, Tensor(a!)? out_hi, Tensor(b!)? out_lo, Tensor(c!)? out_f32) -> ()");
    m.def("conv2d_fwd_x3_affine(Tensor? x_hi, Tensor? x_lo, Tensor? w_hi, Tensor? w_lo, int N, int H, int W, int Cin, int Cout, int kh, int kw, int stride, int pad, Tensor? scale, Tensor? shift, int relu, Tensor(a!)? out_f32, Tensor(b!)? out_hi, Tensor(c!)? out_lo) -> ()");
    m.def("conv2d_dgrad_x3_affine(Tensor? dy_hi, Tensor? dy_lo, Tensor? wt_hi, Tensor? wt_lo, int N, int H, int W, int Cin, int Cout, int kh, int kw, int stride, int pad, Tensor? scale, Tensor? shift, int relu, Tensor(a!)? out_f32, Tensor(b!)? out_hi, Tensor(c!)? out_lo) -> ()");
    m.def("conv2d_dgrad_x3_stat_rows(int N, int H, int W, int Cin, int Cout, int kh, int kw, int stride, int pad) -> int");
    m.def("conv2d_dgrad_x3(Tensor? dy_hi, Tensor? dy_lo, Tensor? wt_hi, Tensor? wt_lo, Tensor(a!)? dx, int N, int H, int W, int Cin, int Cout, int kh, int kw, int stride, int pad, Tensor? addend, Tensor(b!)? stats) -> ()");
    m.def("conv2d_dgrad_x3_pair(Tensor? dy_hi, Tensor? dy_lo, Tensor? wt_hi, Tensor? wt_lo, Tensor? dy2_hi, Tensor? dy2_lo, Tensor? wt2_hi, Tensor? wt2_lo, Tensor(a!)? dx, int N, int H, int W, int Cin, int Cout, int kh, int kw, int pad, Tensor? addend) -> ()");
    m.def("conv2d_dgrad_x3_pair_bn_rows(int N, int H, int W, int Cin, int Cout, int kh, int kw, int pad) -> int");
    m.def("conv2d_dgrad_x3_pair_bn(Tensor? dy_hi, Tensor? dy_lo, Tensor? wt_hi, Tensor? wt_lo, Tensor? dy2_hi, Tensor? dy2_lo, Tensor? wt2_hi, Tensor? wt2_lo, Tensor(a!)? dz, int N, int H, int W, int Cin, int Cout, int kh, int kw, int pad, Tensor? bn_y, Tensor? bn_out_hi, Tensor? bnp, Tensor(b!)? bn_part) -> ()");
    m.def("conv2d_dgrad_x3_bn_rows(int N, int H, int W, int Cin, int Cout, int kh, int kw, int stride, int pad) -> int");
    m.def("conv2d_dgrad_x3_bn(Tensor? dy_hi, Tensor? dy_lo, Tensor? wt_hi, Tensor? wt_lo, Tensor(a!)? dz, int N, int H, int W, int Cin, int Cout, int kh, int kw, int stride, int pad, Tensor? addend, Tensor? bn_y, Tensor? bn_out_hi, Tensor? bnp, Tensor(b!)? bn_part) -> ()");
    m.def("conv2d_wgrad_x3_workspace(int N, int H, int W, int Cin, int Cout, int kh, int kw, int stride, int pad) -> int");
    m.def("conv2d_wgrad_x3(Tensor? x_hi, Tensor? x_lo, Tensor? dy_hi, Tensor? dy_lo, Tensor(a!)? dw, int N, int H, int W, int Cin, int Cout, int kh, int kw, int stride, int pad, Tensor(b!)? workspace, int accumulate) -> ()");
    m.def("conv2d_stem_x3_stat_rows(int N, int H, int W) -> int");
    m.def("conv2d_stem_fwd_x3(Tensor? xpad_hi, Tensor? xpad_lo, Tensor? w_hi, Tensor? w_lo, Tensor(a!)? y, int N, int H, int W, int Cout, Tensor(b!)? stats) -> ()");
    m.def("conv2d_stem_wgrad_x3(Tensor? xpad_hi, Tensor? xpad_lo, Tensor? dy_hi, Tensor? dy_lo, Tensor(a!)? dw, int N, int H, int W, int Cout, Tensor(b!)? workspace) -> ()");
    m.def("bn_apply_x3(Tensor? y, Tensor? res, Tensor? bnp, int M, int C, int relu, Tensor(a!)? out, Tensor(b!)? out_hi, Tensor(c!)? out_lo) -> ()");
    m.def("bn_apply_x3_resbn(Tensor? y, Tensor? res_y, Tensor? bnp, Tensor? res_bnp, int M, int C, int relu, Tensor(a!)? out, Tensor(b!)? out_hi, Tensor(c!)? out_lo) -> ()");
    m.def("bn_apply_x3_respl(Tensor? y, Tensor? res_hi, Tensor? res_lo, Tensor? bnp, int M, int C, int relu, Tensor(a!)? out, Tensor(b!)? out_hi, Tensor(c!)? out_lo) -> ()");
    m.def("bn_fin_apply_x3_ok(int nparts, int C) -> int");
    m.def("bn_fin_apply_x3(Tensor? part, int nparts, int count, Tensor? gamma, Tensor? beta, float eps, float momentum, Tensor(a!)? running_mean, Tensor(b!)? running_var, Tensor(c!)? bnp, Tensor? y, Tensor? res, Tensor? res_hi, Tensor? res_lo, Tensor? res_bnp, int M, int C, int relu, Tensor(d!)? out, Tensor(e!)? out_hi, Tensor(f!)? out_lo) -> ()");
    m.def("bn_bwd_x3(Tensor? dout, Tensor? out, int out_is_hi_plane, Tensor? y, Tensor? bnp, int M, int C, int relu, Tensor(a!)? part, int nparts_given, Tensor(b!)? bwdp, Tensor(c!)? dgamma, Tensor(d!)? dbeta, Tensor(e!)? dy_hi, Tensor(f!)? dy_lo, Tensor(g!)? dz_out) -> ()");
    m.def("col_stats_nparts(int M) -> int");
    m.def("col_stats(Tensor? x, int dtype, int M, int C, Tensor(a!)? part) -> ()");
    m.def("bn_finalize(Tensor? part, int nparts, int C, int count, Tensor? gamma, Tensor? beta, float eps, float momentum, Tensor(a!)? running_mean, Tensor(b!)? running_var, Tensor(c!)? bnp) -> ()");
    m.def("bn_eval_params(int C, Tensor? gamma, Tensor? beta, Tensor? rm, Tensor? rv, float eps, Tensor(a!)? bnp) -> ()");
    m.def("bn_eval_params_batch(Tensor? flat, Tensor? stats, Tensor? desc_dev, int n, int max_c, float eps, Tensor(a!)? out) -> ()");
    m.def("bn_apply(Tensor? y, Tensor? res, Tensor? bnp, int dtype, int M, int C, int relu, Tensor(a!)? out) -> ()");
    m.def("bn_bwd(Tensor? dout, Tensor? out, Tensor? y, Tensor? bnp, int dtype, int M, int C, int relu, Tensor(a!)? part, Tensor(b!)? bwdp, Tensor(c!)? dgamma, Tensor(d!)? dbeta, Tensor(e!)? dy, Tensor(f!)? dz_out) -> ()");
    m.def("relu_bwd(Tensor? dout, Tensor? out, int dtype, int n, Tensor(a!)? dz) -> ()");
    m.def("col_sum(Tensor? x, int dtype, int M, int C, Tensor(a!)? part, Tensor(b!)? out) -> ()");
    m.def("col_sum_x3(Tensor? hi, Tensor? lo, int M, int C, Tensor(a!)? part, Tensor(b!)? out) -> ()");
    m.def("add(Tensor? a, Tensor? b, int dtype, int n, Tensor(a!)? out) -> ()");
    m.def("maxpool3x3s2_fwd(Tensor? x, int dtype, int N, int H, int W, int C, Tensor(a!)? out, Tensor(b!)? idx) -> ()");
    m.def("conv2d_dgrad_bnstats_rows(int dtype, int N, int H, int W, int Cin, int Cout, int kh, int kw, int stride, int pad) -> int");
    m.def("conv2d_dgrad_bnstats(Tensor? dy, Tensor? wt, Tensor(a!)? dx, int dtype, int N, int H, int W, int Cin, int Cout, int kh, int kw, int stride, int pad, Tensor? addend, Tensor? bn_y, Tensor? bn_out, Tensor? bnp, Tensor(b!)? bn_part) -> ()");
    m.def("bn_bwd_apply(Tensor? dout, Tensor? out, Tensor? y, Tensor? bnp, int dtype, int M, int C, int relu, Tensor? part, int nparts, Tensor(a!)? bwdp, Tensor(b!)? dgamma, Tensor(c!)? dbeta, Tensor(d!)? dy, Tensor(e!)? dz_out) -> ()");
    m.def("bn_relu_maxpool3x3s2_fwd(Tensor? y, Tensor? bnp, int dtype, int N, int H, int W, int C, Tensor(a!)? out, Tensor(b!)? idx) -> ()");
    m.def("bn_relu_maxpool3x3s2_fwd_x3(Tensor? y, Tensor? bnp, int N, int H, int W, int C, Tensor(a!)? out, Tensor(b!)? out_hi, Tensor(c!)? out_lo, Tensor(d!)? idx) -> ()");
    m.def("bn_relu_maxpool_bwd(Tensor? dpool, Tensor? idx, Tensor? y, Tensor? bnp, int dtype, int N, int H, int W, int C, Tensor(a!)? part, Tensor(b!)? bwdp, Tensor(c!)? dgamma, Tensor(d!)? dbeta, Tensor(e!)? dy) -> ()");
    m.def("bn_relu_maxpool_bwd_x3_nparts(int N, int H, int W, int C) -> int");
    m.def("bn_relu_maxpool_bwd_x3(Tensor? dpool, Tensor? idx, Tensor? y, Tensor? bnp, int N, int H, int W, int C, Tensor(a!)? part, Tensor(b!)? bwdp, Tensor(c!)? dgamma, Tensor(d!)? dbeta, Tensor(e!)? dz, Tensor(f!)? dy_hi, Tensor(g!)? dy_lo) -> ()");
    m.def("bn_relu_maxpool3x3s2_fwd_x3w(Tensor? y, Tensor? bnp, int N, int H, int W, int C, Tensor(a!)? out, Tensor(b!)? out_hi, Tensor(c!)? out_lo, Tensor(d!)? idx, Tensor(e!)? ywin) -> ()");
    m.def("bn_relu_maxpool_bwd_x3w(Tensor? dpool, Tensor? idx, Tensor? ywin, Tensor? y, Tensor? bnp, int N, int H, int W, int C, Tensor(a!)? part, Tensor(b!)? bwdp, Tensor(c!)? dgamma, Tensor(d!)? dbeta, Tensor(e!)? dy_hi, Tensor(f!)? dy_lo) -> ()");
    m.def("maxpool3x3s2_bwd(Tensor? idx, Tensor? dout, int dtype, int N, int H, int W, int C, Tensor(a!)? dx) -> ()");
    m.def("avgpool_fwd(Tensor? x, int dtype, int N, int HW, int C, Tensor(a!)? out) -> ()");
// ... 77 lines not shown
    m.impl("conv2d_stem_fwd", &w_conv2d_stem_fwd);
    m.impl("conv2d_dgrad_stat_rows", &w_conv2d_dgrad_stat_rows);
    m.impl("conv2d_dgrad", &w_conv2d_dgrad);
    m.impl("conv2d_wgrad_workspace", &w_conv2d_wgrad_workspace);
    m.impl("conv2d_wgrad", &w_conv2d_wgrad);
    m.impl("conv2d_wgrad_deferred", &w_conv2d_wgrad_deferred);
    m.impl("conv2d_stem_wgrad_deferred", &w_conv2d_stem_wgrad_deferred);
    m.impl("conv2d_wgrad_x3_deferred", &w_conv2d_wgrad_x3_deferred);
    m.impl("conv2d_stem_wgrad_x3_deferred", &w_conv2d_stem_wgrad_x3_deferred);
    m.impl("wgrad_reduce_batch", &w_wgrad_reduce_batch);
    m.impl("conv2d_wgrad_x3_group_workspace", &w_conv2d_wgrad_x3_group_workspace);
    m.impl("conv2d_wgrad_x3_group", &w_conv2d_wgrad_x3_group);
    m.impl("conv2d_stem_wgrad_workspace", &w_conv2d_stem_wgrad_workspace);
    m.impl("conv2d_stem_wgrad", &w_conv2d_stem_wgrad);
    m.impl("split_f32", &w_split_f32);
    m.impl("conv2d_x3_stat_rows", &w_conv2d_x3_stat_rows);
    m.impl("conv2d_fwd_x3", &w_conv2d_fwd_x3);
    m.impl("conv1x1_sam_fwd_x3_ok", &w_conv1x1_sam_fwd_x3_ok);
    m.impl("conv1x1_sam_fwd_x3", &w_conv1x1_sam_fwd_x3);
    m.impl("softargmax3d_stage2", &w_softargmax3d_stage2);
    m.impl("conv2d_fwd_x3_evalbn_ok", &w_conv2d_fwd_x3_evalbn_ok);
    m.impl("conv2d_fwd_x3_evalbn", &w_conv2d_fwd_x3_evalbn);
    m.impl("conv2d_fwd_x3_affine", &w_conv2d_fwd_x3_affine);
    m.impl("conv2d_dgrad_x3_affine", &w_conv2d_dgrad_x3_affine);
    m.impl("conv2d_dgrad_x3_stat_rows", &w_conv2d_dgrad_x3_stat_rows);
    m.impl("conv2d_dgrad_x3", &w_conv2d_dgrad_x3);
    m.impl("conv2d_dgrad_x3_pair", &w_conv2d_dgrad_x3_pair);
    m.impl("conv2d_dgrad_x3_pair_bn_rows", &w_conv2d_dgrad_x3_pair_bn_rows);
    m.impl("conv2d_dgrad_x3_pair_bn", &w_conv2d_dgrad_x3_pair_bn);
    m.impl("conv2d_dgrad_x3_bn_rows", &w_conv2d_dgrad_x3_bn_rows);
    m.impl("conv2d_dgrad_x3_bn", &w_conv2d_dgrad_x3_bn);
    m.impl("conv2d_wgrad_x3_workspace", &w_conv2d_wgrad_x3_workspace);
    m.impl("conv2d_wgrad_x3", &w_conv2d_wgrad_x3);
    m.impl("conv2d_stem_x3_stat_rows", &w_conv2d_stem_x3_stat_rows);
    m.impl("conv2d_stem_fwd_x3", &w_conv2d_stem_fwd_x3);
    m.impl("conv2d_stem_wgrad_x3", &w_conv2d_stem_wgrad_x3);
    m.impl("bn_apply_x3", &w_bn_apply_x3);
    m.impl("bn_apply_x3_resbn", &w_bn_apply_x3_resbn);
    m.impl("bn_apply_x3_respl", &w_bn_apply_x3_respl);
    m.impl("bn_fin_apply_x3_ok", &w_bn_fin_apply_x3_ok);
    m.impl("bn_fin_apply_x3", &w_bn_fin_apply_x3);
    m.impl("bn_bwd_x3", &w_bn_bwd_x3);
    m.impl("col_stats_nparts", &w_col_stats_nparts);
    m.impl("col_stats", &w_col_stats);
    m.impl("bn_finalize", &w_bn_finalize);
    m.impl("bn_eval_params", &w_bn_eval_params);
    m.impl("bn_eval_params_batch", &w_bn_eval_params_batch);
    m.impl("bn_apply", &w_bn_apply);
    m.impl("bn_bwd", &w_bn_bwd);
    m.impl("relu_bwd", &w_relu_bwd);
    m.impl("col_sum", &w_col_sum);
    m.impl("col_sum_x3", &w_col_sum_x3);
    m.impl("add", &w_add);
    m.impl("maxpool3x3s2_fwd", &w_maxpool3x3s2_fwd);
    m.impl("conv2d_dgrad_bnstats_rows", &w_conv2d_dgrad_bnstats_rows);
    m.impl("conv2d_dgrad_bnstats", &w_conv2d_dgrad_bnstats);
    m.impl("bn_bwd_apply", &w_bn_bwd_apply);
    m.impl("bn_relu_maxpool3x3s2_fwd", &w_bn_relu_maxpool3x3s2_fwd);
    m.impl("bn_relu_maxpool3x3s2_fwd_x3", &w_bn_relu_maxpool3x3s2_fwd_x3);
    m.impl("bn_relu_maxpool_bwd", &w_bn_relu_maxpool_bwd);
    m.impl("bn_relu_maxpool_bwd_x3_nparts", &w_bn_relu_maxpool_bwd_x3_nparts);
    m.impl("bn_relu_maxpool_bwd_x3", &w_bn_relu_maxpool_bwd_x3);
    m.impl("bn_relu_maxpool3x3s2_fwd_x3w", &w_bn_relu_maxpool3x3s2_fwd_x3w);
    m.impl("bn_relu_maxpool_bwd_x3w", &w_bn_relu_maxpool_bwd_x3w);
    m.impl("maxpool3x3s2_bwd", &w_maxpool3x3s2_bwd);
    m.impl("avgpool_fwd", &w_avgpool_fwd);
// ... 62 lines not shown
```

artiboost_amd/csrc/wgrad.h:

```cpp
#pragma once
#include "common.h"

int wgrad3x3_slices(int N, int H, int W, int Cin, int Cout);
int wgrad3x3_run(const void* x, const void* dy, float* slabs, int N, int H, int W, int Cin, int Cout, hipStream_t st);
int wgrad3x3_x3_group_slices(int G, int N, int H, int W, int Cin, int Cout);
int wgrad3x3_x3_group_run(int G, const void* const* x_hi, const void* const* x_lo, const void* const* dy_hi, const void* const* dy_lo,
                          float* const* slabs, int N, int H, int W, int Cin, int Cout, hipStream_t st);

int wgrad_gemm2_slices(int M, int Cout, int Cin, int ntaps);
int wgrad_gemm2_max_slices(int M, int Cout, int jtot);
int wgrad_gemm2_run(const void* x, const void* dy, float* slabs, int N, int H, int W, int Cin, int Cout, int kh, int kw,
                    int stride, int pad, hipStream_t st);
int wgrad_gemm2_stem_slices(int N, int H, int W, int Cout);
int wgrad_gemm2_stem_run(const void* xpad, const void* dy, float* slabs, int N, int H, int W, int Cout, hipStream_t st);
int wgrad_gemm2_x3_slices(int M, int Cout, int Cin, int ntaps);
int wgrad_gemm2_x3_run(const void* x_hi, const void* x_lo, const void* dy_hi, const void* dy_lo, float* slabs, int N, int H, int W,
                       int Cin, int Cout, int kh, int kw, int stride, int pad, hipStream_t st);
int wgrad_gemm2_x3_stem_run(const void* xpad_hi, const void* xpad_lo, const void* dy_hi, const void* dy_lo, float* slabs, int N,
                            int H, int W, int Cout, hipStream_t st);

int wgrad_launch_reduce(const float* slabs, int ns, long slab_elems, int src_j, int dst_j, float* dst, int accumulate,
                        int stem_mask, hipStream_t st);
void wgrad_reduce_now();

template <class Run>
static inline int wgrad_then_reduce(Run&& run, float* slabs, int ns, int Cout, int src_j, int dst_j, float* dw, int accumulate,
                                    int stem_mask, hipStream_t st) {
    if (int rc = run()) return rc;
    return wgrad_launch_reduce(slabs, ns, (long)Cout * src_j, src_j, dst_j, dw, accumulate, stem_mask, st);
}

static inline int wgrad_rows_per_slice(int M, int n, int step) { return ((M + n - 1) / n + step - 1) / step * step; }

template <class Args>
static inline void wgrad_fill_conv(Args& g, const void* x, const void* dy, float* slabs, int N, int H, int W, int Cin, int Cout, int kh,
                                   int kw, int stride, int pad) {
    g.X = x; g.DY = dy; g.slabs = slabs;
    g.N = N; g.Ha = H; g.Wa = W; g.Ca = Cin;
    g.P = (H + 2 * pad - kh) / stride + 1; g.Q = (W + 2 * pad - kw) / stride + 1; g.Cout = Cout;
    g.stride = stride; g.ntaps = kh * kw; g.Cin = Cin; g.jtot = kh * kw * Cin; g.M = N * g.P * g.Q;
// ... 11 lines not shown
```

artiboost_amd/hybridnet.py:

```python
from collections import OrderedDict

import os

import torch

from . import kernels as K
from .head import softargmax3d_fwd, softargmax3d_bwd, softargmax3d_bwd_x3, softargmax3d_stage2

RESNET34_LAYERS = [3, 4, 6, 3]
DEPTH_PITCH = 32
BOX_OUT_PAD = 64


class _Entry:
    __slots__ = ("name", "kind", "ref_shape", "kshape", "offset", "numel", "bn")

    def __init__(self, name, kind, ref_shape, kshape):
        self.name, self.kind, self.ref_shape, self.kshape = name, kind, tuple(ref_shape), tuple(kshape)
        self.numel = 1
        for d in kshape:
            self.numel *= d
        self.offset = 0


# ... 739 lines not shown
        self._wgrad(dd2, e1, 4, 4, 2, 1, out=gv(hp + ".deconv_layers.3.weight"))
        de1 = self._conv_fwd(dd2, hp + ".deconv_layers.3.weight", 2, 1)
        dd1 = self._bn_bwd(de1, e1, S["d1"], S["bnpd1"], gv(hp + ".deconv_layers.1.weight"),
                       gv(hp + ".deconv_layers.1.bias"), relu="recompute")
        self._wgrad(dd1, feat, 4, 4, 2, 1, out=gv(hp + ".deconv_layers.0.weight"))
        dout = self._conv_fwd(dd1, hp + ".deconv_layers.0.weight", 2, 1)
        if g_mean is not None:
            K.avgpool_bwd(g_mean, dout, accumulate=True)
        blocks = list(reversed(S["blocks"]))
        if stage == 0:
            n4 = sum(1 for r in blocks if r["pre"].startswith("backbone.layer4."))
            dout, part = self._backward_blocks(dout, blocks[:n4], below=blocks[n4] if n4 < len(blocks) else None)
            S["_dout"], S["_blocks_left"], S["_dout_part"] = dout, blocks[n4:], part
            self._wgrad_join()
            return
        self._backward_trunk(S, dout, blocks)

    def _backward_blocks(self, dout, blocks, dout_part=None, below=None):
        gv = self.p.gview
        for k, rec in enumerate(blocks):
            pre, stride, x = rec["pre"], rec["stride"], rec["x"]
            nxt = blocks[k + 1] if k + 1 < len(blocks) else below
            if rec.get("kind") == "bottleneck":
                dout, dout_part = self._bottleneck_bwd(dout, rec, dout_part, nxt)
                continue
            fz = self._frozen(pre)
            dy2, dz = self._bn_bwd(dout, rec["out"], rec["y2"], rec["bnp2"], gv(pre + ".bn2.weight"), gv(pre + ".bn2.bias"),
                               relu=True, want_dz=True, part=dout_part, frozen=fz)
            self._wgrad(rec["a1"], dy2, 3, 3, 1, 1, out=gv(pre + ".conv2.weight"))
            da1, part1 = self._conv_dgrad(dy2, pre + ".conv2.weight", (dy2.shape[-3], dy2.shape[-2]), 1, 1,
                                          bn=(rec["y1"], None, rec["bnp1"]))
            dy1 = self._bn_bwd(da1, rec["a1"], rec["y1"], rec["bnp1"], gv(pre + ".bn1.weight"), gv(pre + ".bn1.bias"),
                            relu="recompute", part=part1, frozen=fz)
            self._wgrad(x, dy1, 3, 3, stride, 1, out=gv(pre + ".conv1.weight"))
            bn_below = (nxt["y2"], nxt["out"], nxt["bnp2"]) if nxt is not None else None
            if rec["ds"]:
                dyd = self._bn_bwd(dz, None, rec["yd"], rec["bnpd"], gv(pre + ".downsample.1.weight"),
                               gv(pre + ".downsample.1.bias"), relu=False, frozen=fz)
                self._wgrad(x, dyd, 1, 1, stride, 0, out=gv(pre + ".downsample.0.weight"))
                if self.x3 and stride == 2:
                    dout = K.conv2d_dgrad_x3_pair(dy1, self.tr[pre + ".conv1.weight"], dyd, self.tr[pre + ".downsample.0.weight"],
                                                  (x.shape[-3], x.shape[-2]), 1, bn=bn_below)
                    dout, dout_part = dout if isinstance(dout, tuple) else (dout, None)
                else:
                    dx = self._conv_dgrad(dy1, pre + ".conv1.weight", (x.shape[-3], x.shape[-2]), stride, 1)
                    dout = self._conv_dgrad(dyd, pre + ".downsample.0.weight", (x.shape[-3], x.shape[-2]), stride, 0, addend=dx)
                    dout_part = None
            elif bn_below is not None:
                dout, dout_part = self._conv_dgrad(dy1, pre + ".conv1.weight", (x.shape[-3], x.shape[-2]), stride, 1,
                                                   addend=dz, bn=bn_below)
            else:
                dout = self._conv_dgrad(dy1, pre + ".conv1.weight", (x.shape[-3], x.shape[-2]), stride, 1, addend=dz)
                dout_part = None
        return dout, dout_part

    def _backward_trunk(self, S, dout, blocks, dout_part=None):
        gv = self.p.gview
        dout, _ = self._backward_blocks(dout, blocks, dout_part)
        y0, dy0 = S["y0"], None
        if self.x3 and not self.frozen_bn:
            dy0 = K.bn_relu_maxpool_bwd_x3(dout, S["pool_idx"], y0, S["bnp0"], gv("backbone.bn1.weight"), gv("backbone.bn1.bias"),
                                           ywin=S.get("pool_ywin"))
        if dy0 is None:
            da0 = K.maxpool_bwd(S["pool_idx"], dout, (y0.shape[1], y0.shape[2]))
            dy0 = self._bn_bwd(da0, None, y0, S["bnp0"], gv("backbone.bn1.weight"), gv("backbone.bn1.bias"), relu="recompute",
                               frozen=self.frozen_bn)
        self._stem_wgrad(S["xpad"], dy0, *S["HW"], out=gv("backbone.conv1.weight"))
        self._wgrad_join()
        self.saved = None
```

artiboost_amd/kernels.py:

```python
import ctypes

import torch

from . import _lib as L


def _empty(shape, like, dtype=None):
    return torch.empty(shape, dtype=dtype or like.dtype, device=like.device)


def conv_out(h, k, s, p):
    return (h + 2 * p - k) // s + 1


def conv2d_fwd(x, w_ohwi, stride, pad, bias=None, want_stats=False, relu=False):
    N, H, W, Cin = x.shape
    Cout, kh, kw, _ = w_ohwi.shape
    Ho, Wo = conv_out(H, kh, stride, pad), conv_out(W, kw, stride, pad)
    y = _empty((N, Ho, Wo, Cout), x)
    lib = L.lib()
    stats = None
    if want_stats:
        nt = lib.ab_conv2d_stat_rows(L.i(L.dt(x)), L.i(N), L.i(H), L.i(W), L.i(Cin), L.i(Cout), L.i(kh), L.i(kw), L.i(stride), L.i(pad), L.i(0))
        stats = torch.empty((nt, Cout, 2), dtype=torch.float32, device=x.device)
# ... 520 lines not shown
                                   L.stream()), "ab_conv2d_dgrad_x3")
    if want_stats:
        return dx, (part if part is not None else col_stats(dx))
    return (dx, None) if bn is not None else dx


def conv2d_dgrad_x3_pair(dy, wt_split, dy2, wt2_split, in_hw, pad, addend=None, bn=None):
    dh, dl = _planes(dy)
    eh, el = _planes(dy2)
    N, Ho, Wo, Cout = dh.shape
    _, Cin, kh, kw, _ = wt_split.shape
    assert tuple(eh.shape) == tuple(dh.shape) and tuple(wt2_split.shape[1:]) == (Cin, 1, 1, Cout)
    H, W = in_hw
    dx = torch.empty((N, H, W, Cin), dtype=torch.float32, device=dh.device)
    lib = L.lib()
    if bn is not None and addend is None:
        bn_y, bn_out, bnp = bn
        rows = lib.ab_conv2d_dgrad_x3_pair_bn_rows(L.i(N), L.i(H), L.i(W), L.i(Cin), L.i(Cout), L.i(kh), L.i(kw), L.i(pad))
        mask, has_mask = _relu_mask(bn_out)
        if rows > 0 and has_mask:
            part = torch.empty((rows, Cin, 2), dtype=torch.float32, device=dh.device)
            L.check(lib.ab_conv2d_dgrad_x3_pair_bn(L.ptr(dh), L.ptr(dl), L.ptr(wt_split[0]), L.ptr(wt_split[1]), L.ptr(eh), L.ptr(el),
                                                   L.ptr(wt2_split[0]), L.ptr(wt2_split[1]), L.ptr(dx), L.i(N), L.i(H), L.i(W), L.i(Cin),
                                                   L.i(Cout), L.i(kh), L.i(kw), L.i(pad), L.ptr(bn_y), L.ptr(mask), L.ptr(bnp), L.ptr(part),
                                                   L.stream()), "ab_conv2d_dgrad_x3_pair_bn")
            return dx, part
    L.check(lib.ab_conv2d_dgrad_x3_pair(L.ptr(dh), L.ptr(dl), L.ptr(wt_split[0]), L.ptr(wt_split[1]), L.ptr(eh), L.ptr(el),
                                        L.ptr(wt2_split[0]), L.ptr(wt2_split[1]), L.ptr(dx), L.i(N), L.i(H), L.i(W), L.i(Cin),
                                        L.i(Cout), L.i(kh), L.i(kw), L.i(pad), L.ptr(addend), L.stream()),
            "ab_conv2d_dgrad_x3_pair")
    return (dx, None) if bn is not None else dx


def conv2d_wgrad_x3(x, dy, kh, kw, stride, pad, out=None, accumulate=False, defer=None):
    xh, xl = _planes(x)
    dh, dl = _planes(dy)
    N, H, W, Cin = xh.shape
    Cout = dh.shape[3]
    lib = L.lib()
    nbytes = lib.ab_conv2d_wgrad_x3_workspace(L.i(N), L.i(H), L.i(W), L.i(Cin), L.i(Cout), L.i(kh), L.i(kw), L.i(stride), L.i(pad))
    if nbytes <= 0:
        raise RuntimeError(f"conv2d_wgrad_x3: shape not handled (Cin {Cin}, Cout {Cout}, {kh}x{kw})")
    dw = out if out is not None else torch.empty((Cout, kh, kw, Cin), dtype=torch.float32, device=xh.device)
    if defer is not None:
        ws, d = defer.new(nbytes, xh.device)
        L.check(lib.ab_conv2d_wgrad_x3_deferred(L.ptr(xh), L.ptr(xl), L.ptr(dh), L.ptr(dl), L.ptr(dw), L.i(N), L.i(H), L.i(W), L.i(Cin),
                                                L.i(Cout), L.i(kh), L.i(kw), L.i(stride), L.i(pad), L.ptr(ws), L.i(1 if accumulate else 0),
                                                ctypes.byref(d), L.stream()), "ab_conv2d_wgrad_x3_deferred")
        return dw
    ws = _workspace(nbytes, xh.device)
    L.check(lib.ab_conv2d_wgrad_x3(L.ptr(xh), L.ptr(xl), L.ptr(dh), L.ptr(dl), L.ptr(dw), L.i(N), L.i(H), L.i(W), L.i(Cin),
                                   L.i(Cout), L.i(kh), L.i(kw), L.i(stride), L.i(pad), L.ptr(ws), L.i(1 if accumulate else 0),
                                   L.stream()), "ab_conv2d_wgrad_x3")
    return dw


WGRAD_GROUP_MAX = 8


def conv2d_wgrad_x3_group_ok(x, dy, G):
    xh, dh = _planes(x)[0], _planes(dy)[0]
    N, H, W, Cin = xh.shape
    return dh.shape[:3] == xh.shape[:3] and 1 <= G <= WGRAD_GROUP_MAX and \
        L.lib().ab_conv2d_wgrad_x3_group_workspace(L.i(G), L.i(N), L.i(H), L.i(W), L.i(Cin), L.i(dh.shape[3])) > 0


def conv2d_wgrad_x3_group(items, accumulate=False):
    G = len(items)
    planes = [(_planes(x), _planes(dy), out) for x, dy, out in items]
    (xh, _), (dh, _), _ = planes[0]
    N, H, W, Cin = xh.shape
    Cout = dh.shape[3]
    lib = L.lib()
    nbytes = lib.ab_conv2d_wgrad_x3_group_workspace(L.i(G), L.i(N), L.i(H), L.i(W), L.i(Cin), L.i(Cout))
    if nbytes <= 0:
        raise RuntimeError(f"conv2d_wgrad_x3_group: shape not handled ({G} x [{N},{H},{W},{Cin}] -> {Cout})")
    arr = (L.WgradGroupItem * G)()
    for i, ((a, b), (c, d), out) in enumerate(planes):
        assert a.shape == xh.shape and c.shape == dh.shape and out.dtype == torch.float32 and out.numel() == Cout * 9 * Cin and out.is_contiguous()
        arr[i].x_hi, arr[i].x_lo, arr[i].dy_hi, arr[i].dy_lo, arr[i].dw = a.data_ptr(), b.data_ptr(), c.data_ptr(), d.data_ptr(), out.data_ptr()
    ws = _workspace(nbytes, xh.device)
    L.check(lib.ab_conv2d_wgrad_x3_group(arr, L.i(G), L.i(N), L.i(H), L.i(W), L.i(Cin), L.i(Cout), L.ptr(ws), L.i(1 if accumulate else 0),
                                         L.stream()), "ab_conv2d_wgrad_x3_group")
    return [out for _, _, out in planes]


def bn_apply_x3(y, bnp, res=None, relu=True, want_f32=False, res_bnp=None):
# ... 483 lines not shown
```

include/artiboost_hip.h:

```cpp
#ifndef ARTIBOOST_HIP_H
#define ARTIBOOST_HIP_H
#include <stdint.h>
#ifdef __cplusplus
extern "C" {
#endif

#define AB_DT_F32 0
#define AB_DT_BF16 1
#define AB_DT_U8N 2
#define AB_EINVAL (-1)
#define AB_ESHAPE (-2)
#define AB_EALIGN (-3)

int ab_abi_version(void);

int ab_wall_stamp(int64_t* slot, void* stream);
int ab_wall_clock_khz(void);

int ab_softargmax3d_ntiles(int H, int W);
int ab_softargmax3d_fwd(const void* logits, int dtype, int B, int C, int D, int DP, int H, int W,
                        float* part, float* uvd, float* conf, float* stat, void* stream);
int ab_softargmax3d_bwd(const void* logits, int dtype, int B, int C, int D, int DP, int H, int W,
                        const float* uvd, const float* conf, const float* stat,
                        const float* g_uvd, const float* g_conf, void* dlogits, void* stream);
// ... 65 lines not shown
int ab_conv1x1_sam_fwd_x3(const void* x_hi, const void* x_lo, const void* w_hi, const void* w_lo, const float* bias, float* logits,
                          int B, int H, int W, int Cin, int C, int D, float* part, void* stream);
int ab_softargmax3d_stage2(const float* part, int B, int C, int ntile, float* uvd, float* conf, float* stat, void* stream);
int ab_conv2d_fwd_x3_evalbn_ok(int N, int H, int W, int Cin, int Cout);
int ab_conv2d_fwd_x3_evalbn(const void* x_hi, const void* x_lo, const void* w_hi, const void* w_lo, int N, int H, int W, int Cin,
                            int Cout, const float* bnp, const void* res_hi, const void* res_lo, const float* res_f32, int relu,
                            void* out_hi, void* out_lo, float* out_f32, void* stream);
int ab_conv2d_fwd_x3_affine(const void* x_hi, const void* x_lo, const void* w_hi, const void* w_lo, int N, int H, int W, int Cin,
                            int Cout, int kh, int kw, int stride, int pad, const float* scale, const float* shift, int relu,
                            float* out_f32, void* out_hi, void* out_lo, void* stream);
int ab_conv2d_dgrad_x3_affine(const void* dy_hi, const void* dy_lo, const void* wt_hi, const void* wt_lo, int N, int H, int W, int Cin,
                              int Cout, int kh, int kw, int stride, int pad, const float* scale, const float* shift, int relu,
                              float* out_f32, void* out_hi, void* out_lo, void* stream);
int ab_conv2d_dgrad_x3_stat_rows(int N, int H, int W, int Cin, int Cout, int kh, int kw, int stride, int pad);
int ab_conv2d_dgrad_x3(const void* dy_hi, const void* dy_lo, const void* wt_hi, const void* wt_lo, float* dx, int N, int H,
                       int W, int Cin, int Cout, int kh, int kw, int stride, int pad, const float* addend, float* stats,
                       void* stream);
int ab_conv2d_dgrad_x3_pair(const void* dy_hi, const void* dy_lo, const void* wt_hi, const void* wt_lo, const void* dy2_hi,
                            const void* dy2_lo, const void* wt2_hi, const void* wt2_lo, float* dx, int N, int H, int W, int Cin,
                            int Cout, int kh, int kw, int pad, const float* addend, void* stream);
int ab_conv2d_dgrad_x3_pair_bn_rows(int N, int H, int W, int Cin, int Cout, int kh, int kw, int pad);
int ab_conv2d_dgrad_x3_pair_bn(const void* dy_hi, const void* dy_lo, const void* wt_hi, const void* wt_lo, const void* dy2_hi,
                               const void* dy2_lo, const void* wt2_hi, const void* wt2_lo, float* dz, int N, int H, int W, int Cin,
                               int Cout, int kh, int kw, int pad, const float* bn_y, const void* bn_out_hi, const float* bnp,
                               float* bn_part, void* stream);
int ab_conv2d_dgrad_x3_bn_rows(int N, int H, int W, int Cin, int Cout, int kh, int kw, int stride, int pad);
int ab_conv2d_dgrad_x3_bn(const void* dy_hi, const void* dy_lo, const void* wt_hi, const void* wt_lo, float* dz, int N, int H,
                          int W, int Cin, int Cout, int kh, int kw, int stride, int pad, const float* addend,
                          const float* bn_y, const void* bn_out_hi, const float* bnp, float* bn_part, void* stream);
long ab_conv2d_wgrad_x3_workspace(int N, int H, int W, int Cin, int Cout, int kh, int kw, int stride, int pad);
int ab_conv2d_wgrad_x3(const void* x_hi, const void* x_lo, const void* dy_hi, const void* dy_lo, float* dw, int N, int H,
                       int W, int Cin, int Cout, int kh, int kw, int stride, int pad, void* workspace, int accumulate,
                       void* stream);

int ab_conv2d_stem_x3_stat_rows(int N, int H, int W);
int ab_conv2d_stem_fwd_x3(const void* xpad_hi, const void* xpad_lo, const void* w_hi, const void* w_lo, float* y, int N, int H,
                          int W, int Cout, float* stats, void* stream);
int ab_conv2d_stem_wgrad_x3(const void* xpad_hi, const void* xpad_lo, const void* dy_hi, const void* dy_lo, float* dw, int N,
                            int H, int W, int Cout, void* workspace, void* stream);
int ab_bn_apply_x3(const float* y, const float* res, const float* bnp, long M, int C, int relu, float* out, void* out_hi,
                   void* out_lo, void* stream);
int ab_bn_apply_x3_resbn(const float* y, const float* res_y, const float* bnp, const float* res_bnp, long M, int C, int relu,
                         float* out, void* out_hi, void* out_lo, void* stream);
int ab_bn_apply_x3_respl(const float* y, const void* res_hi, const void* res_lo, const float* bnp, long M, int C, int relu,
                         float* out, void* out_hi, void* out_lo, void* stream);
int ab_bn_fin_apply_x3_ok(int nparts, int C);
int ab_bn_fin_apply_x3(const float* part, int nparts, long count, const float* gamma, const float* beta, float eps, float momentum,
                       float* running_mean, float* running_var, float* bnp, const float* y, const float* res, const void* res_hi,
                       const void* res_lo, const float* res_bnp, long M, int C, int relu, float* out, void* out_hi, void* out_lo,
                       void* stream);
int ab_bn_bwd_x3(const float* dout, const void* out, int out_is_hi_plane, const float* y, const float* bnp, long M, int C,
                 int relu, float* part, int nparts_given, float* bwdp, float* dgamma, float* dbeta, void* dy_hi, void* dy_lo,
                 float* dz_out, void* stream);

int ab_col_stats_nparts(long M);
int ab_col_stats(const void* x, int dtype, long M, int C, float* part, void* stream);
int ab_bn_finalize(const float* part, int nparts, int C, long count, const float* gamma, const float* beta,
                   float eps, float momentum, float* running_mean, float* running_var, float* bnp, void* stream);
int ab_bn_eval_params(int C, const float* gamma, const float* beta, const float* rm, const float* rv, float eps,
                      float* bnp, void* stream);
int ab_bn_eval_params_batch(const float* flat, const float* stats, const int32_t* desc_dev, int n, int max_c, float eps, float* out,
                            void* stream);
int ab_bn_apply(const void* y, const void* res, const float* bnp, int dtype, long M, int C, int relu, void* out,
                void* stream);
int ab_bn_bwd(const void* dout, const void* out, const void* y, const float* bnp, int dtype, long M, int C, int relu,
              float* part, float* bwdp, float* dgamma, float* dbeta, void* dy, void* dz_out, void* stream);
// ... 252 lines not shown
```

Before: 7668 samples/s.

## Fuse stride-2 3x3 and downsample 1x1 weight gradients into one kernel

Result: no change. 7724 samples/s (median of 6 runs) (+0.7%).

```diff
diff --git a/artiboost_amd/csrc/conv_x3.hip b/artiboost_amd/csrc/conv_x3.hip
--- a/artiboost_amd/csrc/conv_x3.hip
+++ b/artiboost_amd/csrc/conv_x3.hip
@@ -372,6 +372,29 @@
                              slabs, ns, Cout, jtot, jtot, dw, accumulate, 0, st);
 }
 
+extern "C" long ab_conv2d_wgrad_x3_s2_workspace(int N, int H, int W, int Cin, int Cout) {
+    const int ns = wgrad3x3s2_slices(N, H, W, Cin, Cout);
+    return ns > 0 ? (long)ns * Cout * 10 * Cin * 4 : 0;
+}
+extern "C" int ab_conv2d_wgrad_x3_s2(const void* x_hi, const void* x_lo, const void* dy_hi, const void* dy_lo, float* dw,
+                                     const void* dyd_hi, const void* dyd_lo, float* dwd, int N, int H, int W, int Cin, int Cout,
+                                     void* workspace, int accumulate, void* stream) {
+    const int ns = wgrad3x3s2_slices(N, H, W, Cin, Cout);
+    if (!ns) return AB_ESHAPE;
+    if (!x_hi || !x_lo || !dy_hi || !dy_lo || !dw || !workspace) return AB_EINVAL;
+    if (!dyd_hi != !dyd_lo || !dyd_hi != !dwd) return AB_EINVAL;
+    const long slab3 = (long)Cout * 9 * Cin, slabd = (long)Cout * Cin;
+    const bool direct = ns == 1 && !accumulate;
+    float* const s3 = direct ? dw : (float*)workspace;
+    float* const sd = direct ? dwd : (float*)workspace + ns * slab3;
+    int rc = wgrad3x3s2_run(x_hi, x_lo, dy_hi, dy_lo, dyd_hi, dyd_lo, s3, sd, N, H, W, Cin, Cout, as_stream(stream));
+    if (rc || direct) return rc;
+    ab_wgrad_reduce_desc d[2] = {};
+    d[0].slabs = s3; d[0].dst = dw; d[0].slab_elems = slab3; d[0].nslices = ns; d[0].src_j = d[0].dst_j = 9 * Cin; d[0].accumulate = accumulate;
+    d[1].slabs = sd; d[1].dst = dwd; d[1].slab_elems = slabd; d[1].nslices = ns; d[1].src_j = d[1].dst_j = Cin; d[1].accumulate = accumulate;
+    return ab_wgrad_reduce_batch(d, dyd_hi ? 2 : 1, stream);
+}
+
 extern "C" int ab_conv2d_stem_x3_stat_rows(int N, int H, int W) {
     if (int t = stem_halo_x3_tiles(N, H, W)) return t;
     return conv_gemm2_x3_stem_mtiles(N * (H / 2) * (W / 2));
diff --git a/artiboost_amd/csrc/torch_ops_gen.cpp b/artiboost_amd/csrc/torch_ops_gen.cpp
--- a/artiboost_amd/csrc/torch_ops_gen.cpp
+++ b/artiboost_amd/csrc/torch_ops_gen.cpp
@@ -87,6 +87,8 @@
 static void w_conv2d_dgrad_x3_bn(const c10::optional<at::Tensor>& dy_hi, const c10::optional<at::Tensor>& dy_lo, const c10::optional<at::Tensor>& wt_hi, const c10::optional<at::Tensor>& wt_lo, const c10::optional<at::Tensor>& dz, int64_t N, int64_t H, int64_t W, int64_t Cin, int64_t Cout, int64_t kh, int64_t kw, int64_t stride, int64_t pad, const c10::optional<at::Tensor>& addend, const c10::optional<at::Tensor>& bn_y, const c10::optional<at::Tensor>& bn_out_hi, const c10::optional<at::Tensor>& bnp, const c10::optional<at::Tensor>& bn_part) { static const char* const OP = "artiboost_hip::conv2d_dgrad_x3_bn"; ck_dev(OP, "dy_hi", dy_hi, (int)-1, true); ck_dev(OP, "dy_lo", dy_lo, (int)-1, true); ck_dev(OP, "wt_hi", wt_hi, (int)-1, true); ck_dev(OP, "wt_lo", wt_lo, (int)-1, true); ck_dev(OP, "dz", dz, (int)at::kFloat, true); ck_dev(OP, "addend", addend, (int)at::kFloat, true); ck_dev(OP, "bn_y", bn_y, (int)at::kFloat, true); ck_dev(OP, "bn_out_hi", bn_out_hi, (int)-1, true); ck_dev(OP, "bnp", bnp, (int)at::kFloat, true); ck_dev(OP, "bn_part", bn_part, (int)at::kFloat, true); ck_dtype(OP, "dy_hi", dy_hi, at::kBFloat16); ck_dtype(OP, "dy_lo", dy_lo, at::kBFloat16); ck_dtype(OP, "wt_hi", wt_hi, at::kBFloat16); ck_dtype(OP, "wt_lo", wt_lo, at::kBFloat16); ck_dtype(OP, "bn_out_hi", bn_out_hi, at::kBFloat16); ck_numel(OP, "dy_hi", dy_hi, (int64_t)(N*co(H,kh,stride,pad)*co(W,kw,stride,pad)*Cout)); ck_numel(OP, "dy_lo", dy_lo, (int64_t)(N*co(H,kh,stride,pad)*co(W,kw,stride,pad)*Cout)); ck_numel(OP, "wt_hi", wt_hi, (int64_t)(Cin*kh*kw*Cout)); ck_numel(OP, "wt_lo", wt_lo, (int64_t)(Cin*kh*kw*Cout)); ck_numel(OP, "dz", dz, (int64_t)(N*H*W*Cin)); ck_numel(OP, "addend", addend, (int64_t)(N*H*W*Cin)); ck_numel(OP, "bn_y", bn_y, (int64_t)(N*H*W*Cin)); ck_numel(OP, "bn_out_hi", bn_out_hi, (int64_t)(N*H*W*Cin)); ck_numel(OP, "bnp", bnp, (int64_t)(4*Cin)); ck_numel(OP, "bn_part", bn_part, (int64_t)(ab_conv2d_dgrad_x3_bn_rows(N,H,W,Cin,Cout,kh,kw,stride,pad)*Cin*2)); const long rc = (long)ab_conv2d_dgrad_x3_bn((const void*)p(dy_hi), (const void*)p(dy_lo), (const void*)p(wt_hi), (const void*)p(wt_lo), (float*)p(dz), (int)N, (int)H, (int)W, (int)Cin, (int)Cout, (int)kh, (int)kw, (int)stride, (int)pad, (const float*)p(addend), (const float*)p(bn_y), (const void*)p(bn_out_hi), (const float*)p(bnp), (float*)p(bn_part), cur_stream()); TORCH_CHECK(rc == 0, "ab_conv2d_dgrad_x3_bn failed with code ", rc, rc > 0 ? " (hipError)" : " (argument error)"); }
 static int64_t w_conv2d_wgrad_x3_workspace(int64_t N, int64_t H, int64_t W, int64_t Cin, int64_t Cout, int64_t kh, int64_t kw, int64_t stride, int64_t pad) { return (int64_t)ab_conv2d_wgrad_x3_workspace((int)N, (int)H, (int)W, (int)Cin, (int)Cout, (int)kh, (int)kw, (int)stride, (int)pad); }
 static void w_conv2d_wgrad_x3(const c10::optional<at::Tensor>& x_hi, const c10::optional<at::Tensor>& x_lo, const c10::optional<at::Tensor>& dy_hi, const c10::optional<at::Tensor>& dy_lo, const c10::optional<at::Tensor>& dw, int64_t N, int64_t H, int64_t W, int64_t Cin, int64_t Cout, int64_t kh, int64_t kw, int64_t stride, int64_t pad, const c10::optional<at::Tensor>& workspace, int64_t accumulate) { static const char* const OP = "artiboost_hip::conv2d_wgrad_x3"; ck_dev(OP, "x_hi", x_hi, (int)-1, true); ck_dev(OP, "x_lo", x_lo, (int)-1, true); ck_dev(OP, "dy_hi", dy_hi, (int)-1, true); ck_dev(OP, "dy_lo", dy_lo, (int)-1, true); ck_dev(OP, "dw", dw, (int)at::kFloat, true); ck_dev(OP, "workspace", workspace, (int)-1, true); ck_dtype(OP, "x_hi", x_hi, at::kBFloat16); ck_dtype(OP, "x_lo", x_lo, at::kBFloat16); ck_dtype(OP, "dy_hi", dy_hi, at::kBFloat16); ck_dtype(OP, "dy_lo", dy_lo, at::kBFloat16); ck_numel(OP, "x_hi", x_hi, (int64_t)(N*H*W*Cin)); ck_numel(OP, "x_lo", x_lo, (int64_t)(N*H*W*Cin)); ck_numel(OP, "dy_hi", dy_hi, (int64_t)(N*co(H,kh,stride,pad)*co(W,kw,stride,pad)*Cout)); ck_numel(OP, "dy_lo", dy_lo, (int64_t)(N*co(H,kh,stride,pad)*co(W,kw,stride,pad)*Cout)); ck_numel(OP, "dw", dw, (int64_t)(Cout*kh*kw*Cin)); ck_bytes(OP, "workspace", workspace, (int64_t)(ab_conv2d_wgrad_x3_workspace(N,H,W,Cin,Cout,kh,kw,stride,pad))); const long rc = (long)ab_conv2d_wgrad_x3((const void*)p(x_hi), (const void*)p(x_lo), (const void*)p(dy_hi), (const void*)p(dy_lo), (float*)p(dw), (int)N, (int)H, (int)W, (int)Cin, (int)Cout, (int)kh, (int)kw, (int)stride, (int)pad, (void*)p(workspace), (int)accumulate, cur_stream()); TORCH_CHECK(rc == 0, "ab_conv2d_wgrad_x3 failed with code ", rc, rc > 0 ? " (hipError)" : " (argument error)"); }
+static int64_t w_conv2d_wgrad_x3_s2_workspace(int64_t N, int64_t H, int64_t W, int64_t Cin, int64_t Cout) { return (int64_t)ab_conv2d_wgrad_x3_s2_workspace((int)N, (int)H, (int)W, (int)Cin, (int)Cout); }
+static void w_conv2d_wgrad_x3_s2(const c10::optional<at::Tensor>& x_hi, const c10::optional<at::Tensor>& x_lo, const c10::optional<at::Tensor>& dy_hi, const c10::optional<at::Tensor>& dy_lo, const c10::optional<at::Tensor>& dw, const c10::optional<at::Tensor>& dyd_hi, const c10::optional<at::Tensor>& dyd_lo, const c10::optional<at::Tensor>& dwd, int64_t N, int64_t H, int64_t W, int64_t Cin, int64_t Cout, const c10::optional<at::Tensor>& workspace, int64_t accumulate) { static const char* const OP = "artiboost_hip::conv2d_wgrad_x3_s2"; ck_dev(OP, "x_hi", x_hi, (int)-1, true); ck_dev(OP, "x_lo", x_lo, (int)-1, true); ck_dev(OP, "dy_hi", dy_hi, (int)-1, true); ck_dev(OP, "dy_lo", dy_lo, (int)-1, true); ck_dev(OP, "dw", dw, (int)at::kFloat, true); ck_dev(OP, "dyd_hi", dyd_hi, (int)-1, true); ck_dev(OP, "dyd_lo", dyd_lo, (int)-1, true); ck_dev(OP, "dwd", dwd, (int)at::kFloat, true); ck_dev(OP, "workspace", workspace, (int)-1, true); ck_dtype(OP, "x_hi", x_hi, at::kBFloat16); ck_dtype(OP, "x_lo", x_lo, at::kBFloat16); ck_dtype(OP, "dy_hi", dy_hi, at::kBFloat16); ck_dtype(OP, "dy_lo", dy_lo, at::kBFloat16); ck_dtype(OP, "dyd_hi", dyd_hi, at::kBFloat16); ck_dtype(OP, "dyd_lo", dyd_lo, at::kBFloat16); ck_numel(OP, "x_hi", x_hi, (int64_t)(N*H*W*Cin)); ck_numel(OP, "x_lo", x_lo, (int64_t)(N*H*W*Cin)); ck_numel(OP, "dy_hi", dy_hi, (int64_t)(N*(H/2)*(W/2)*Cout)); ck_numel(OP, "dy_lo", dy_lo, (int64_t)(N*(H/2)*(W/2)*Cout)); ck_numel(OP, "dyd_hi", dyd_hi, (int64_t)(N*(H/2)*(W/2)*Cout)); ck_numel(OP, "dyd_lo", dyd_lo, (int64_t)(N*(H/2)*(W/2)*Cout)); ck_numel(OP, "dw", dw, (int64_t)(Cout*9*Cin)); ck_numel(OP, "dwd", dwd, (int64_t)(Cout*Cin)); ck_bytes(OP, "workspace", workspace, (int64_t)(ab_conv2d_wgrad_x3_s2_workspace(N,H,W,Cin,Cout))); const long rc = (long)ab_conv2d_wgrad_x3_s2((const void*)p(x_hi), (const void*)p(x_lo), (const void*)p(dy_hi), (const void*)p(dy_lo), (float*)p(dw), (const void*)p(dyd_hi), (const void*)p(dyd_lo), (float*)p(dwd), (int)N, (int)H, (int)W, (int)Cin, (int)Cout, (void*)p(workspace), (int)accumulate, cur_stream()); TORCH_CHECK(rc == 0, "ab_conv2d_wgrad_x3_s2 failed with code ", rc, rc > 0 ? " (hipError)" : " (argument error)"); }
 static int64_t w_conv2d_stem_x3_stat_rows(int64_t N, int64_t H, int64_t W) { return (int64_t)ab_conv2d_stem_x3_stat_rows((int)N, (int)H, (int)W); }
 static void w_conv2d_stem_fwd_x3(const c10::optional<at::Tensor>& xpad_hi, const c10::optional<at::Tensor>& xpad_lo, const c10::optional<at::Tensor>& w_hi, const c10::optional<at::Tensor>& w_lo, const c10::optional<at::Tensor>& y, int64_t N, int64_t H, int64_t W, int64_t Cout, const c10::optional<at::Tensor>& stats) { static const char* const OP = "artiboost_hip::conv2d_stem_fwd_x3"; ck_dev(OP, "xpad_hi", xpad_hi, (int)-1, true); ck_dev(OP, "xpad_lo", xpad_lo, (int)-1, true); ck_dev(OP, "w_hi", w_hi, (int)-1, true); ck_dev(OP, "w_lo", w_lo, (int)-1, true); ck_dev(OP, "y", y, (int)at::kFloat, true); ck_dev(OP, "stats", stats, (int)at::kFloat, true); ck_dtype(OP, "xpad_hi", xpad_hi, at::kBFloat16); ck_dtype(OP, "xpad_lo", xpad_lo, at::kBFloat16); ck_dtype(OP, "w_hi", w_hi, at::kBFloat16); ck_dtype(OP, "w_lo", w_lo, at::kBFloat16); ck_numel(OP, "xpad_hi", xpad_hi, (int64_t)(N*(H+6)*(W+8)*4)); ck_numel(OP, "xpad_lo", xpad_lo, (int64_t)(N*(H+6)*(W+8)*4)); ck_numel(OP, "w_hi", w_hi, (int64_t)(Cout*7*8*4)); ck_numel(OP, "w_lo", w_lo, (int64_t)(Cout*7*8*4)); ck_numel(OP, "y", y, (int64_t)(N*(H/2)*(W/2)*Cout)); ck_numel(OP, "stats", stats, (int64_t)(ab_conv2d_stem_x3_stat_rows(N,H,W)*Cout*2)); const long rc = (long)ab_conv2d_stem_fwd_x3((const void*)p(xpad_hi), (const void*)p(xpad_lo), (const void*)p(w_hi), (const void*)p(w_lo), (float*)p(y), (int)N, (int)H, (int)W, (int)Cout, (float*)p(stats), cur_stream()); TORCH_CHECK(rc == 0, "ab_conv2d_stem_fwd_x3 failed with code ", rc, rc > 0 ? " (hipError)" : " (argument error)"); }
 static void w_conv2d_stem_wgrad_x3(const c10::optional<at::Tensor>& xpad_hi, const c10::optional<at::Tensor>& xpad_lo, const c10::optional<at::Tensor>& dy_hi, const c10::optional<at::Tensor>& dy_lo, const c10::optional<at::Tensor>& dw, int64_t N, int64_t H, int64_t W, int64_t Cout, const c10::optional<at::Tensor>& workspace) { static const char* const OP = "artiboost_hip::conv2d_stem_wgrad_x3"; ck_dev(OP, "xpad_hi", xpad_hi, (int)-1, true); ck_dev(OP, "xpad_lo", xpad_lo, (int)-1, true); ck_dev(OP, "dy_hi", dy_hi, (int)-1, true); ck_dev(OP, "dy_lo", dy_lo, (int)-1, true); ck_dev(OP, "dw", dw, (int)at::kFloat, true); ck_dev(OP, "workspace", workspace, (int)-1, true); ck_dtype(OP, "xpad_hi", xpad_hi, at::kBFloat16); ck_dtype(OP, "xpad_lo", xpad_lo, at::kBFloat16); ck_dtype(OP, "dy_hi", dy_hi, at::kBFloat16); ck_dtype(OP, "dy_lo", dy_lo, at::kBFloat16); ck_numel(OP, "xpad_hi", xpad_hi, (int64_t)(N*(H+6)*(W+8)*4)); ck_numel(OP, "xpad_lo", xpad_lo, (int64_t)(N*(H+6)*(W+8)*4)); ck_numel(OP, "dy_hi", dy_hi, (int64_t)(N*(H/2)*(W/2)*Cout)); ck_numel(OP, "dy_lo", dy_lo, (int64_t)(N*(H/2)*(W/2)*Cout)); ck_numel(OP, "dw", dw, (int64_t)(Cout*7*8*4)); const long rc = (long)ab_conv2d_stem_wgrad_x3((const void*)p(xpad_hi), (const void*)p(xpad_lo), (const void*)p(dy_hi), (const void*)p(dy_lo), (float*)p(dw), (int)N, (int)H, (int)W, (int)Cout, (void*)p(workspace), cur_stream()); TORCH_CHECK(rc == 0, "ab_conv2d_stem_wgrad_x3 failed with code ", rc, rc > 0 ? " (hipError)" : " (argument error)"); }
@@ -275,6 +277,8 @@
     m.def("conv2d_dgrad_x3_bn(Tensor? dy_hi, Tensor? dy_lo, Tensor? wt_hi, Tensor? wt_lo, Tensor(a!)? dz, int N, int H, int W, int Cin, int Cout, int kh, int kw, int stride, int pad, Tensor? addend, Tensor? bn_y, Tensor? bn_out_hi, Tensor? bnp, Tensor(b!)? bn_part) -> ()");
     m.def("conv2d_wgrad_x3_workspace(int N, int H, int W, int Cin, int Cout, int kh, int kw, int stride, int pad) -> int");
     m.def("conv2d_wgrad_x3(Tensor? x_hi, Tensor? x_lo, Tensor? dy_hi, Tensor? dy_lo, Tensor(a!)? dw, int N, int H, int W, int Cin, int Cout, int kh, int kw, int stride, int pad, Tensor(b!)? workspace, int accumulate) -> ()");
+    m.def("conv2d_wgrad_x3_s2_workspace(int N, int H, int W, int Cin, int Cout) -> int");
+    m.def("conv2d_wgrad_x3_s2(Tensor? x_hi, Tensor? x_lo, Tensor? dy_hi, Tensor? dy_lo, Tensor(a!)? dw, Tensor? dyd_hi, Tensor? dyd_lo, Tensor(b!)? dwd, int N, int H, int W, int Cin, int Cout, Tensor(c!)? workspace, int accumulate) -> ()");
     m.def("conv2d_stem_x3_stat_rows(int N, int H, int W) -> int");
     m.def("conv2d_stem_fwd_x3(Tensor? xpad_hi, Tensor? xpad_lo, Tensor? w_hi, Tensor? w_lo, Tensor(a!)? y, int N, int H, int W, int Cout, Tensor(b!)? stats) -> ()");
     m.def("conv2d_stem_wgrad_x3(Tensor? xpad_hi, Tensor? xpad_lo, Tensor? dy_hi, Tensor? dy_lo, Tensor(a!)? dw, int N, int H, int W, int Cout, Tensor(b!)? workspace) -> ()");
@@ -418,6 +422,8 @@
     m.impl("conv2d_dgrad_x3_bn", &w_conv2d_dgrad_x3_bn);
     m.impl("conv2d_wgrad_x3_workspace", &w_conv2d_wgrad_x3_workspace);
     m.impl("conv2d_wgrad_x3", &w_conv2d_wgrad_x3);
+    m.impl("conv2d_wgrad_x3_s2_workspace", &w_conv2d_wgrad_x3_s2_workspace);
+    m.impl("conv2d_wgrad_x3_s2", &w_conv2d_wgrad_x3_s2);
     m.impl("conv2d_stem_x3_stat_rows", &w_conv2d_stem_x3_stat_rows);
     m.impl("conv2d_stem_fwd_x3", &w_conv2d_stem_fwd_x3);
     m.impl("conv2d_stem_wgrad_x3", &w_conv2d_stem_wgrad_x3);
diff --git a/artiboost_amd/csrc/wgrad.h b/artiboost_amd/csrc/wgrad.h
--- a/artiboost_amd/csrc/wgrad.h
+++ b/artiboost_amd/csrc/wgrad.h
@@ -6,6 +6,10 @@
 int wgrad3x3_x3_group_slices(int G, int N, int H, int W, int Cin, int Cout);
 int wgrad3x3_x3_group_run(int G, const void* const* x_hi, const void* const* x_lo, const void* const* dy_hi, const void* const* dy_lo,
                           float* const* slabs, int N, int H, int W, int Cin, int Cout, hipStream_t st);
+
+int wgrad3x3s2_slices(int N, int H, int W, int Cin, int Cout);
+int wgrad3x3s2_run(const void* x_hi, const void* x_lo, const void* dy_hi, const void* dy_lo, const void* dyd_hi, const void* dyd_lo,
+                   float* out3, float* outd, int N, int H, int W, int Cin, int Cout, hipStream_t st);
 
 int wgrad_gemm2_slices(int M, int Cout, int Cin, int ntaps);
 int wgrad_gemm2_max_slices(int M, int Cout, int jtot);
diff --git a/artiboost_amd/csrc/wgrad3x3s2.hip b/artiboost_amd/csrc/wgrad3x3s2.hip
--- /dev/null
+++ b/artiboost_amd/csrc/wgrad3x3s2.hip
@@ -0,0 +1,223 @@
+#include "wgrad_common.h"
+#include "wgrad.h"
+
+struct Wg3s2Args {
+    const void* X; const void* X_lo; const void* DY; const void* DY_lo; const void* DYD; const void* DYD_lo;
+    float* out3; float* outd;
+    int N, H, Cin, Cout;
+    int bands_per_slice, nbands;
+    int xcd_map;
+};
+
+static constexpr int wg3s2_r8(int n) { return (n + 7) / 8 * 8; }
+
+template <int WO, int TH>
+__global__ __launch_bounds__(512) void wgrad3x3s2_kernel(Wg3s2Args g) {
+    constexpr int NW = 8;
+    constexpr int BP = TH * WO;
+    static_assert(BP == 32, "bands of 32 output pixels");
+    constexpr int KS = BP / 16;
+    constexpr int PWE = WO, PWO = WO + 4;
+    constexpr int RE = TH, RO = TH + 1;
+    constexpr int SG0 = 0, SG1 = SG0 + wg3s2_r8(RE * PWE), SG2 = SG1 + wg3s2_r8(RE * PWO), SG3 = SG2 + wg3s2_r8(RO * PWE);
+    constexpr int NPIX = SG3 + wg3s2_r8(RO * PWO);
+    constexpr int IA = BP / 8, IX = NPIX / 8;
+    constexpr int NF = 4 * IA + 2 * IX;
+    constexpr int LF = (NF + NW - 1) / NW;
+    constexpr int ABYTES = IA * 1024, XBYTES = IX * 1024, BUF = NF * 1024;
+    extern __shared__ __attribute__((aligned(16))) unsigned char smem[];
+    const unsigned lds0 = lds_addr_of(smem);
+
+    const int tid = threadIdx.x, lane = tid & 63, wave = __builtin_amdgcn_readfirstlane(tid >> 6);
+    const int tiles_ci = g.Cin / 64;
+    int bx, by; xcd_slice_major(g.xcd_map, bx, by);
+    const int tile_co = bx / tiles_ci, tile_ci = bx - tile_co * tiles_ci;
+    const int co0 = tile_co * 64, ci0 = tile_ci * 64;
+    const int wco = (wave & 1) * 32, wci = ((wave >> 1) & 1) * 32;
+    const int tg = wave >> 2;
+    const bool has_ds = g.DYD != nullptr;
+    const int band_begin = by * g.bands_per_slice;
+    const int band_end = min(g.nbands, band_begin + g.bands_per_slice);
+    const int bands_per_img = (g.H / 2) / TH;
+    const int W = 2 * WO;
+    const bf16_t* zp = (const bf16_t*)wg_zero_page;
+
+    const bf16_t* f_src[LF]; long f_off[LF]; bool f_on[LF], f_isx[LF], f_ok[LF], f_top[LF];
+#pragma unroll
+    for (int j = 0; j < LF; ++j) {
+        const int f = wave + NW * j;
+        f_on[j] = f < NF; f_isx[j] = f >= 4 * IA; f_ok[j] = true; f_top[j] = false;
+        if (!f_isx[j]) {
+            const int t = f / IA, ii = f - t * IA;
+            const int p = ii * 8 + (lane >> 3);
+            f_src[j] = (const bf16_t*)(t == 0 ? g.DY : t == 1 ? g.DY_lo : t == 2 ? g.DYD : g.DYD_lo);
+            if (t >= 2 && !has_ds) f_on[j] = false;
+            f_off[j] = (long)p * g.Cout + co0 + swz_chunk<128>(p, lane & 7) * 8;
+        } else {
+            const int fx = f - 4 * IA;
+            const int pl = fx >= IX ? 1 : 0, ii = fx - pl * IX;
+            const int q = ii * 8 + (lane >> 3);
+            const int sg = q >= SG3 ? 3 : q >= SG2 ? 2 : q >= SG1 ? 1 : 0;
+            const int ql = q - (sg == 3 ? SG3 : sg == 2 ? SG2 : sg == 1 ? SG1 : SG0);
+            const int oddc = sg & 1, oddr = sg >> 1;
+            const int pitch = oddc ? PWO : PWE, rows = oddr ? RO : RE;
+            const int pr = ql / pitch, pc = ql - pr * pitch;
+            f_ok[j] = pr < rows && (!oddc || (pc >= 1 && pc <= WO));
+            f_top[j] = oddr && pr == 0;
+            f_src[j] = (const bf16_t*)(pl ? g.X_lo : g.X);
+            const int row = 2 * pr - oddr, col = 2 * pc - oddc;
+            f_off[j] = ((long)row * W + col) * g.Cin + ci0 + swz_chunk<128>(q, lane & 7) * 8;
+        }
+    }
+    auto issue_band = [&](int band, int buf) {
+        const int img = band / bands_per_img, y0 = (band - img * bands_per_img) * TH;
+        const long dsh = (((long)img * (g.H / 2) + y0) * WO) * g.Cout;
+        const long xsh = (((long)img * g.H + 2 * y0) * W) * g.Cin;
+#pragma unroll
+        for (int j = 0; j < LF; ++j) {
+            if (!f_on[j]) continue;
+            const bool ok = f_ok[j] && !(f_top[j] && y0 == 0);
+            const bf16_t* s = f_src[j] + (f_isx[j] ? xsh : dsh) + f_off[j];
+            glds16(ok ? s : zp, __builtin_amdgcn_readfirstlane(lds0 + buf * BUF + (wave + NW * j) * 1024));
+        }
+    };
+
+    const int grp = lane >> 4, l16 = lane & 15;
+    const int krow = (grp >> 1) * 8 + (l16 >> 2);
+    const int csub = (grp & 1) * 16 + (l16 & 3) * 4;
+    unsigned a_base[2];
+#pragma unroll
+    for (int h = 0; h < 2; ++h) a_base[h] = frag_addr<128>(krow + h * 4, wco + csub);
+    unsigned x_base[3][2];
+#pragma unroll
+    for (int h = 0; h < 2; ++h) {
+        const int p = krow + h * 4, ty = p / WO, tx = p - ty * WO;
+        x_base[0][h] = frag_addr<128>(ty * PWE + tx, wci + csub);
+        x_base[1][h] = frag_addr<128>(ty * PWO + tx, wci + csub);
+        x_base[2][h] = frag_addr<128>(ty * PWO + tx + 1, wci + csub);
+    }
+
+    f32x16 acc[5];
+#pragma unroll
+    for (int t = 0; t < 5; ++t)
+#pragma unroll
+        for (int r = 0; r < 16; ++r) acc[t][r] = 0.f;
+
+    auto tap_v = [](int t) constexpr { const int kw = t == 9 ? 1 : t % 3; return kw == 1 ? 0 : kw == 2 ? 2 : 1; };
+    auto tap_disp = [](int t, int s) constexpr {
+        const int kh = t == 9 ? 1 : t / 3, kw = t == 9 ? 1 : t % 3, p0 = 16 * s, oy = p0 / WO, ox = p0 % WO;
+        const int pitch = kw == 1 ? PWE : PWO;
+        const int sg0 = kh == 1 ? (kw == 1 ? SG0 : SG1) : (kw == 1 ? SG2 : SG3);
+        return (sg0 + (oy + (kh == 2)) * pitch + ox) * 128;
+    };
+    unsigned x_sel[5][2]; int t_disp[5][KS];
+#pragma unroll
+    for (int tt = 0; tt < 5; ++tt) {
+#pragma unroll
+        for (int h = 0; h < 2; ++h) x_sel[tt][h] = tg ? x_base[tap_v(5 + tt)][h] : x_base[tap_v(tt)][h];
+#pragma unroll
+        for (int s = 0; s < KS; ++s) t_disp[tt][s] = tg ? tap_disp(5 + tt, s) : tap_disp(tt, s);
+    }
+    const unsigned a_ds = tg ? 2 * ABYTES : 0;
+
+    auto band_compute = [&](unsigned sb) {
+        const unsigned xb = sb + 4 * ABYTES;
+#pragma unroll
+        for (int s = 0; s < KS; ++s) {
+            const int p0 = 16 * s;
+            const uint4 fa = tr_pair(sb + a_base[0] + p0 * 128, sb + a_base[1] + p0 * 128);
+            const uint4 fal = tr_pair(sb + ABYTES + a_base[0] + p0 * 128, sb + ABYTES + a_base[1] + p0 * 128);
+#pragma unroll
+            for (int tt = 0; tt < 5; ++tt) {
+                const unsigned d = xb + t_disp[tt][s];
+                const uint4 fb = tr_pair(x_sel[tt][0] + d, x_sel[tt][1] + d);
+                const uint4 fbl = tr_pair(x_sel[tt][0] + d + XBYTES, x_sel[tt][1] + d + XBYTES);
+                if (tt < 4) {
+                    mfma16(acc[tt], fa, fb);
+                    mfma16(acc[tt], fa, fbl);
+                    mfma16(acc[tt], fal, fb);
+                } else {
+                    const unsigned da = sb + a_ds + p0 * 128;
+                    const uint4 fd = tr_pair(da + a_base[0], da + a_base[1]);
+                    const uint4 fdl = tr_pair(da + ABYTES + a_base[0], da + ABYTES + a_base[1]);
+                    mfma16(acc[tt], fd, fb);
+                    mfma16(acc[tt], fd, fbl);
+                    mfma16(acc[tt], fdl, fb);
+                }
+            }
+        }
+    };
+
+    if (band_begin < band_end) issue_band(band_begin, 0);
+    int buf = 0;
+    for (int band = band_begin; band < band_end; ++band) {
+        asm volatile("s_waitcnt vmcnt(0)" ::: "memory");
+        asm volatile("s_waitcnt lgkmcnt(0)" ::: "memory");
+        __builtin_amdgcn_s_barrier();
+        asm volatile("" ::: "memory");
+        if (band + 1 < band_end) issue_band(band + 1, buf ^ 1);
+        const unsigned sb = lds0 + buf * BUF;
+        band_compute(sb);
+        buf ^= 1;
+    }
+    float* out3 = g.out3 + (long)by * g.Cout * 9 * g.Cin;
+#pragma unroll
+    for (int tt = 0; tt < 5; ++tt) {
+        const int t = tg * 5 + tt;
+        if (t < 9) store_acc_tile(out3, 9 * g.Cin, co0 + wco, t * g.Cin + ci0 + wci, acc[tt]);
+        else if (has_ds) store_acc_tile(g.outd + (long)by * g.Cout * g.Cin, g.Cin, co0 + wco, ci0 + wci, acc[tt]);
+    }
+}
+
+template <int WO, int TH>
+static int wg3s2_launch(Wg3s2Args& g, int tiles, int nslices, hipStream_t st) {
+    constexpr int NPIX = wg3s2_r8(TH * WO) + wg3s2_r8(TH * (WO + 4)) + wg3s2_r8((TH + 1) * WO) + wg3s2_r8((TH + 1) * (WO + 4));
+    constexpr size_t lds = (size_t)2 * (4 * (TH * WO / 8) + 2 * (NPIX / 8)) * 1024;
+    static_assert(lds <= 160 * 1024, "two stages in LDS");
+    static bool attr_done = false;
+    if (!attr_done) {
+        hipError_t e = hipFuncSetAttribute((const void*)wgrad3x3s2_kernel<WO, TH>, hipFuncAttributeMaxDynamicSharedMemorySize, (int)lds);
+        if (e != hipSuccess) return (int)e;
+        attr_done = true;
+    }
+    g.xcd_map = 1;
+    wgrad3x3s2_kernel<WO, TH><<<dim3(tiles, nslices), 512, lds, st>>>(g);
+    hipError_t e = hipGetLastError();
+    return e == hipSuccess ? 0 : (int)e;
+}
+
+static int wg3s2_th(int H, int W) {
+    if (H <= 0 || W <= 0 || (H & 1) || (W & 1)) return 0;
+    const int wo = W / 2;
+    if (wo != 32 && wo != 16 && wo != 8) return 0;
+    const int th = 32 / wo;
+    return (H / 2) % th == 0 ? th : 0;
+}
+
+int wgrad3x3s2_slices(int N, int H, int W, int Cin, int Cout) {
+    const int th = wg3s2_th(H, W);
+    if (!th || N <= 0 || Cin <= 0 || Cout <= 0 || Cin % 64 || Cout % 64) return 0;
+    const long tiles = (long)(Cin / 64) * (Cout / 64);
+    if (tiles > 256) return 0;
+    const int nbands = N * ((H / 2) / th);
+    int ns = 256 / (int)tiles;
+    if (ns > nbands / 2) ns = nbands / 2 > 0 ? nbands / 2 : 1;
+    const int bps = (nbands + ns - 1) / ns;
+    return (nbands + bps - 1) / bps;
+}
+
+int wgrad3x3s2_run(const void* x_hi, const void* x_lo, const void* dy_hi, const void* dy_lo, const void* dyd_hi, const void* dyd_lo,
+                   float* out3, float* outd, int N, int H, int W, int Cin, int Cout, hipStream_t st) {
+    const int ns = wgrad3x3s2_slices(N, H, W, Cin, Cout);
+    if (!ns) return AB_ESHAPE;
+    const int th = wg3s2_th(H, W);
+    Wg3s2Args g = {};
+    g.X = x_hi; g.X_lo = x_lo; g.DY = dy_hi; g.DY_lo = dy_lo; g.DYD = dyd_hi; g.DYD_lo = dyd_lo; g.out3 = out3; g.outd = outd;
+    g.N = N; g.H = H; g.Cin = Cin; g.Cout = Cout;
+    g.nbands = N * ((H / 2) / th);
+    g.bands_per_slice = (g.nbands + ns - 1) / ns;
+    const int tiles = (Cin / 64) * (Cout / 64);
+    if (W == 64) return wg3s2_launch<32, 1>(g, tiles, ns, st);
+    if (W == 32) return wg3s2_launch<16, 2>(g, tiles, ns, st);
+    return wg3s2_launch<8, 4>(g, tiles, ns, st);
+}
diff --git a/artiboost_amd/hybridnet.py b/artiboost_amd/hybridnet.py
--- a/artiboost_amd/hybridnet.py
+++ b/artiboost_amd/hybridnet.py
@@ -795,12 +795,17 @@
                                           bn=(rec["y1"], None, rec["bnp1"]))
             dy1 = self._bn_bwd(da1, rec["a1"], rec["y1"], rec["bnp1"], gv(pre + ".bn1.weight"), gv(pre + ".bn1.bias"),
                             relu="recompute", part=part1, frozen=fz)
-            self._wgrad(x, dy1, 3, 3, stride, 1, out=gv(pre + ".conv1.weight"))
+            pair = bool(rec["ds"]) and stride == 2 and self.x3 and not self.wgrad_1pass and K.conv2d_wgrad_x3_s2_ok(x, dy1)
+            if not pair:
+                self._wgrad(x, dy1, 3, 3, stride, 1, out=gv(pre + ".conv1.weight"))
             bn_below = (nxt["y2"], nxt["out"], nxt["bnp2"]) if nxt is not None else None
             if rec["ds"]:
                 dyd = self._bn_bwd(dz, None, rec["yd"], rec["bnpd"], gv(pre + ".downsample.1.weight"),
                                gv(pre + ".downsample.1.bias"), relu=False, frozen=fz)
-                self._wgrad(x, dyd, 1, 1, stride, 0, out=gv(pre + ".downsample.0.weight"))
+                if pair:
+                    K.conv2d_wgrad_x3(x, dy1, 3, 3, 2, 1, out=gv(pre + ".conv1.weight"), pair=(dyd, gv(pre + ".downsample.0.weight")))
+                else:
+                    self._wgrad(x, dyd, 1, 1, stride, 0, out=gv(pre + ".downsample.0.weight"))
                 if self.x3 and stride == 2:
                     dout = K.conv2d_dgrad_x3_pair(dy1, self.tr[pre + ".conv1.weight"], dyd, self.tr[pre + ".downsample.0.weight"],
                                                   (x.shape[-3], x.shape[-2]), 1, bn=bn_below)
diff --git a/artiboost_amd/kernels.py b/artiboost_amd/kernels.py
--- a/artiboost_amd/kernels.py
+++ b/artiboost_amd/kernels.py
@@ -576,7 +576,10 @@
     return (dx, None) if bn is not None else dx
 
 
-def conv2d_wgrad_x3(x, dy, kh, kw, stride, pad, out=None, accumulate=False, defer=None):
+def conv2d_wgrad_x3(x, dy, kh, kw, stride, pad, out=None, accumulate=False, defer=None, pair=None):
+    if pair is not None:
+        assert (kh, kw, stride, pad) == (3, 3, 2, 1) and defer is None
+        return conv2d_wgrad_x3_s2(x, dy, pair[0], out=out, outd=pair[1], accumulate=accumulate)[0]
     xh, xl = _planes(x)
     dh, dl = _planes(dy)
     N, H, W, Cin = xh.shape
@@ -597,6 +600,33 @@
                                    L.i(Cout), L.i(kh), L.i(kw), L.i(stride), L.i(pad), L.ptr(ws), L.i(1 if accumulate else 0),
                                    L.stream()), "ab_conv2d_wgrad_x3")
     return dw
+
+
+def conv2d_wgrad_x3_s2_ok(x, dy):
+    shape = lambda t: tuple(t[0].shape if isinstance(t, tuple) or t.dtype == torch.bfloat16 else t.shape)
+    (N, H, W, Cin), ds = shape(x), shape(dy)
+    return ds[:3] == (N, H // 2, W // 2) and L.lib().ab_conv2d_wgrad_x3_s2_workspace(L.i(N), L.i(H), L.i(W), L.i(Cin), L.i(ds[3])) > 0
+
+
+def conv2d_wgrad_x3_s2(x, dy, dyd=None, out=None, outd=None, accumulate=False):
+    xh, xl = _planes(x)
+    dh, dl = _planes(dy)
+    N, H, W, Cin = xh.shape
+    Cout = dh.shape[3]
+    lib = L.lib()
+    nbytes = lib.ab_conv2d_wgrad_x3_s2_workspace(L.i(N), L.i(H), L.i(W), L.i(Cin), L.i(Cout))
+    if nbytes <= 0 or tuple(dh.shape[:3]) != (N, H // 2, W // 2):
+        raise RuntimeError(f"conv2d_wgrad_x3_s2: shape not handled ([{N},{H},{W},{Cin}] -> {tuple(dh.shape)})")
+    dw = out if out is not None else torch.empty((Cout, 3, 3, Cin), dtype=torch.float32, device=xh.device)
+    eh = el = dwd = None
+    if dyd is not None:
+        eh, el = _planes(dyd)
+        assert eh.shape == dh.shape
+        dwd = outd if outd is not None else torch.empty((Cout, 1, 1, Cin), dtype=torch.float32, device=xh.device)
+    ws = _workspace(nbytes, xh.device)
+    L.check(lib.ab_conv2d_wgrad_x3_s2(L.ptr(xh), L.ptr(xl), L.ptr(dh), L.ptr(dl), L.ptr(dw), L.ptr(eh), L.ptr(el), L.ptr(dwd), L.i(N), L.i(H),
+                                      L.i(W), L.i(Cin), L.i(Cout), L.ptr(ws), L.i(1 if accumulate else 0), L.stream()), "ab_conv2d_wgrad_x3_s2")
+    return dw if dyd is None else (dw, dwd)
 
 
 WGRAD_GROUP_MAX = 8
diff --git a/include/artiboost_hip.h b/include/artiboost_hip.h
--- a/include/artiboost_hip.h
+++ b/include/artiboost_hip.h
@@ -121,6 +121,10 @@
 int ab_conv2d_wgrad_x3(const void* x_hi, const void* x_lo, const void* dy_hi, const void* dy_lo, float* dw, int N, int H,
                        int W, int Cin, int Cout, int kh, int kw, int stride, int pad, void* workspace, int accumulate,
                        void* stream);
+long ab_conv2d_wgrad_x3_s2_workspace(int N, int H, int W, int Cin, int Cout);
+int ab_conv2d_wgrad_x3_s2(const void* x_hi, const void* x_lo, const void* dy_hi, const void* dy_lo, float* dw, const void* dyd_hi,
+                          const void* dyd_lo, float* dwd, int N, int H, int W, int Cin, int Cout, void* workspace, int accumulate,
+                          void* stream);
 
 int ab_conv2d_stem_x3_stat_rows(int N, int H, int W);
 int ab_conv2d_stem_fwd_x3(const void* xpad_hi, const void* xpad_lo, const void* w_hi, const void* w_lo, float* y, int N, int H,
```
